# TheNeodev/RVC-MAKER

Measured on AMD Instinct MI355X. Metric: audio-seconds/sec/GPU (xRT) end-to-end VC, 48k v2; 1/2/4/8 GPU scaling, higher is better.
Workload: dtype f32-equivalent (split-fp16 3-pass MFMA for the generator's convs -- scale from the producer's published |max| -- and ResBlock pairs, split-bf16 6-pass MFMA elsewhere; f32 accumulate; RMVPE f64 with its GRU recurrence f32); 1 GPU; VC.pipeline 48k v2, ContentVec-768, rmvpe f0, one 30 s clip per GPU per step, no index, protect 0.33, clip stream (clip k+1 f0/features under clip k synthesizer); model=RVC v2 48k (NSF-HiFiGAN) + ContentVec + rmvpe, global_batch=1, seq_len=480000, parallelism=utterance-sharded x1

## Files before the change

### include/rvc_amd.h

```cpp
#ifndef RVC_AMD_H
#define RVC_AMD_H

#include <stdint.h>

#ifdef __cplusplus
extern "C" {
#endif

typedef struct ihipStream_t* rvc_stream_t;

enum { RVC_OK = 0, RVC_EINVAL = -22, RVC_EHIP = -5 };

enum {
    RVC_ACT_NONE = 0,
    RVC_ACT_LRELU = 1,
    RVC_ACT_RELU = 2,
    RVC_ACT_TANH = 3,
    RVC_ACT_GELU = 4,
    RVC_ACT_SIGMOID = 5,
    RVC_ACT_LOGCLAMP = 6,
};

const char* rvc_last_error(void);
int rvc_version(void);
// ... 3 lines not shown
#define RVC_ARITH_FP32_SA 7

typedef struct rvc_conv1d_args {
    const float* x;
    const float* w;
    const float* bias;
    const float* bias2;
    const float* res;
    float* y;
    int64_t B, Ci, Co, Lin, Lout;
    int64_t ncols;
    int64_t x_bstride, y_bstride, res_bstride, w_bstride;
    int K, stride, dil, pad, groups;
    int nphase, ostride, ooffset;
    int in_act, out_act, accumulate, _pad0;
    float in_scale, in_slope, out_slope, out_scale;
    int ntoff, wrap;
    int toff[16];
    const void* wx;
    int wx_nmf, wx_passes;
    const unsigned* amax_in;
    unsigned* amax_out;
    const float* src_x;
    const float* src_w;
    const float* src_b;
    int src_K, src_stride, src_pad, _pad1;
    int64_t src_len, src_bstride;
} rvc_conv1d_args;

int64_t rvc_conv1d_workspace_bytes(const rvc_conv1d_args* a);
int rvc_conv1d_engine(const rvc_conv1d_args* a);
int rvc_conv1d_tile(const rvc_conv1d_args* a);
int rvc_conv1d(const rvc_conv1d_args* a, void* ws, int64_t ws_bytes, rvc_stream_t stream);
void rvc_conv1d_set_probe_event(void* hip_event);
int rvc_conv1d_set_stamps(void* buf, int64_t bytes);
int rvc_resblock_set_stamps(void* buf, int64_t bytes);
int rvc_resblock_set_ylds(int on);
int rvc_resblock_set_wide64(int on);
int rvc_conv1d_set_tile_epi(int on);
int rvc_conv1d_set_swz(int on);
int rvc_conv1d_set_f16_fast(int on);
int rvc_conv1d_set_splitk_target(int target);
int rvc_stream_create_cu_mask(const uint32_t* mask, int nwords, rvc_stream_t* out);
int rvc_stream_destroy(rvc_stream_t stream);
int64_t rvc_conv1d_x6_bytes(int64_t nphase, int64_t Ci, int K, int64_t Co);
int rvc_conv1d_pack_x6(const float* w_km, int64_t nphase, int64_t Ci, int K, int64_t Co, void* out, int* nmf_out,
                       rvc_stream_t stream);
int64_t rvc_conv1d_f16_bytes(int64_t nphase, int64_t Ci, int K, int64_t Co);
int rvc_conv1d_pack_f16(const float* w_km, int64_t nphase, int64_t Ci, int K, int64_t Co, void* out, int* nmf_out,
                        rvc_stream_t stream);

typedef struct rvc_resblock_args {
    const float* x;
    float* y;
    const void* w1x;
    const float* b1;
    const void* w2x;
    const float* b2;
    int64_t C, L;
    int K, dil, nmf1, nmf2, passes, accumulate;
    float slope;
    int B;
} rvc_resblock_args;

int64_t rvc_resblock_lds_bytes(int64_t C, int K, int dil, int passes);
int rvc_resblock_pair(const rvc_resblock_args* a, rvc_stream_t stream);

typedef struct rvc_attn_args {
    const float* q;
    const float* k;
    const float* v;
    float* o;
    const float* rk;
    const float* ev;
    float* ml;
    int64_t B, H, D, T;
    int64_t ldc;
    int64_t q_hs, k_hs, v_hs, o_hs;
    int64_t q_bs, k_bs, v_bs, o_bs;
    int W, _pad0;
    float scale, _pad1;
} rvc_attn_args;

int64_t rvc_attention_workspace_bytes(const rvc_attn_args* a);
int rvc_attention(const rvc_attn_args* a, void* ws, int64_t ws_bytes, rvc_stream_t stream);
int rvc_attention_amax(const rvc_attn_args* a, unsigned* amax_out, void* ws, int64_t ws_bytes, rvc_stream_t stream);
int rvc_attention_ex(const rvc_attn_args* a, const unsigned* amax_in, unsigned* amax_out, void* ws, int64_t ws_bytes,
                     rvc_stream_t stream);
int rvc_attention_set_f16(int on);

int rvc_textenc_embed(const float* lin, const float* emb, const int64_t* pitch, float* out, int64_t B, int64_t C,
                      int64_t T, float scale, float slope, rvc_stream_t stream);
int rvc_textenc_embed_amax(const float* lin, const float* emb, const int64_t* pitch, float* out, int64_t B, int64_t C,
                           int64_t T, float scale, float slope, unsigned* amax_out, rvc_stream_t stream);
int rvc_layernorm_cf(const float* x, const float* res, const float* gamma, const float* beta, float* out, int64_t B,
                     int64_t C, int64_t T, float eps, rvc_stream_t stream);
int rvc_layernorm_cf_amax(const float* x, const float* res, const float* gamma, const float* beta, float* out,
                          int64_t B, int64_t C, int64_t T, float eps, unsigned* amax_out, rvc_stream_t stream);
int rvc_chnorm_gelu(const float* x, const float* gamma, const float* beta, float* out, int64_t B, int64_t C, int64_t L,
                    float eps, int gelu, rvc_stream_t stream);
int64_t rvc_fe0_ws_bytes(int64_t B, int64_t C, int64_t T);
int rvc_fe0_gn_gelu(const float* x, int64_t B, int64_t N, int64_t x_bstride, const float* w_km, int64_t C, int K,
                    int stride, const float* gamma, const float* beta, float* out, float eps, int gelu, void* ws,
                    int64_t ws_bytes, rvc_stream_t stream);
int rvc_fe0_gn_gelu_amax(const float* x, int64_t B, int64_t N, int64_t x_bstride, const float* w_km, int64_t C, int K,
                         int stride, const float* gamma, const float* beta, float* out, float eps, int gelu,
                         unsigned* amax_out, void* ws, int64_t ws_bytes, rvc_stream_t stream);
int rvc_prior_sample(const float* stats, const float* noise, float* zp, int64_t B, int64_t C, int64_t T, float nscale,
                     rvc_stream_t stream);
int rvc_gate(const float* a, float* out, int64_t B, int64_t H, int64_t T, rvc_stream_t stream);
int rvc_flip_channels(const float* x, float* out, int64_t B, int64_t C, int64_t T, rvc_stream_t stream);
int rvc_transpose(const float* in, float* out, int64_t B, int64_t R, int64_t C, rvc_stream_t stream);
int rvc_randn(float* out, int64_t n, uint64_t seed, uint64_t offset, rvc_stream_t stream);
int rvc_randn_ex(float* out, int64_t n, uint64_t seed, uint64_t offset, const uint64_t* seed_add,
                 rvc_stream_t stream);
int rvc_rand_triang(float* out, int64_t n, float lo, float hi, uint64_t seed, uint64_t offset,
                    const uint64_t* seed_add, rvc_stream_t stream);
int rvc_sine_source(const float* f0, const float* noise, float* har, float* work, int64_t B, int64_t T, int upp,
                    float sr, float lin_w, float lin_b, rvc_stream_t stream);

#define RVC_HARMONIC_MAX 16
#define RVC_ADAIN_BMAX 16
int rvc_rand_uniform(float* out, int64_t n, uint64_t seed, uint64_t offset, const uint64_t* seed_add,
                     rvc_stream_t stream);
int64_t rvc_harmonic_source_ws_bytes(int64_t B, int64_t T, int upp, int H);
int64_t rvc_harmonic_source_chunk(void);
int rvc_harmonic_source(const float* f0, const float* phase0, const float* noise, float* har, int64_t B, int64_t T,
                        int upp, int H, int linear, float sr, const float* lin_w, float lin_b, void* ws,
                        int64_t ws_bytes, rvc_stream_t stream);
int rvc_upsample_linear(const float* x, float* y, int64_t B, int64_t C, int64_t Lin, int r, int64_t x_bstride,
                        int64_t y_bstride, int act, float slope, rvc_stream_t stream);
int rvc_adain(const float* x, const float* noise, const float* w, float* y, int64_t B, int64_t C, int64_t L,
              float slope, float out_scale, int accumulate, const uint64_t* seeds, uint64_t offset,
              const uint64_t* seed_add, rvc_stream_t stream);

int rvc_stft_frames(const float* x, const float* win, float* framesT, int64_t N, int64_t F, int nfft, int hop,
                    rvc_stream_t stream);
int rvc_spec_mag(const float* spec, float* mag, int64_t K, int64_t F, rvc_stream_t stream);
int rvc_stft_mag(const float* x, const float* win, float* mag, int64_t B, int64_t N, int64_t F, int nfft, int hop,
                 int64_t x_bstride, int64_t mag_bstride, rvc_stream_t stream);
int rvc_mel_image(const float* mel, float* img, int64_t M, int64_t F, int64_t Tp, float scale, float shift,
                  rvc_stream_t stream);
int rvc_avgpool2(const float* in, float* out, int64_t C, int64_t H, int64_t W, rvc_stream_t stream);
// ... 301 lines not shown
```

### rvc-maker_amd/csrc/attention.hip

```cpp
#include "rvc_common.h"
#include "x6_common.h"
#include <stdlib.h>

namespace {

struct AttnParams {
    const float* q;
    const float* k;
    const float* v;
    float* o;
    const float* rk;
    float* ml;
    float* ws;
    int64_t T;
    int64_t ldc;
    int64_t q_hs, k_hs, v_hs, o_hs;
    int64_t q_bs, k_bs, v_bs, o_bs;
    int H, W, S, kps;
    float scale;
    unsigned* amax_out;
    const unsigned* amax_in;
};

template <int D>
// ... 424 lines not shown
    const float* wml = p.ws + (int64_t)gridDim.z * S * p.H * D * T;
    float m = -INFINITY;
    for (int s = 0; s < S; ++s) m = fmaxf(m, wml[(((int64_t)b * S + s) * p.H + h) * 2 * T + q]);
    float wsum = 0.f, acc[NC];
#pragma unroll
    for (int j = 0; j < NC; ++j) acc[j] = 0.f;
    for (int s = 0; s < S; ++s) {
        const int64_t bsh = ((int64_t)b * S + s) * p.H + h;
        const float w = wml[bsh * 2 * T + T + q] * expf(wml[bsh * 2 * T + q] - m);
        wsum += w;
        const float* wo = p.ws + bsh * D * T + q;
#pragma unroll
        for (int j = 0; j < NC; ++j) acc[j] += w * wo[(int64_t)(cg + 4 * j) * T];
    }
    const float inv = 1.f / wsum;
    float* O = p.o + b * p.o_bs + h * p.o_hs;
    float amx = 0.f;
    if (ok) {
#pragma unroll
        for (int j = 0; j < NC; ++j) {
            O[(int64_t)(cg + 4 * j) * p.ldc + q] = acc[j] * inv;
            amx = fmaxf(amx, fabsf(acc[j] * inv));
        }
    }
    if (p.amax_out) amax_publish(p.amax_out + (int64_t)b * RVC_AMAX_SHARDS, amx);
    if (!ok) return;
    if (p.ml && cg == 0) {
        float* ML = p.ml + ((int64_t)b * p.H + h) * 2 * T;
        ML[q] = m;
        ML[T + q] = wsum;
    }
}

constexpr int RELV_QB = 32, RELV_KW = RELV_QB + 2 * 15;
__global__ __launch_bounds__(256) void attn_relv_band_kernel(AttnParams p, const float* ev, int D) {
    constexpr int QB = RELV_QB;
    __shared__ float pb[QB][32];
    __shared__ float evs[31 * 96];
    __shared__ float qs[96][QB + 1];
    __shared__ float ks[96][RELV_KW + 1];
    const int h = blockIdx.y, b = blockIdx.z;
    const int64_t T = p.T;
    const int64_t q0 = (int64_t)blockIdx.x * QB;
    const int tid = threadIdx.x;
    const int nb = 2 * p.W + 1, kw = QB + 2 * p.W;
    const float* Q = p.q + b * p.q_bs + h * p.q_hs;
    const float* K = p.k + b * p.k_bs + h * p.k_hs;
    const float* RK = p.rk + ((int64_t)b * p.H + h) * nb * T;
    const float* ML = p.ml + ((int64_t)b * p.H + h) * 2 * T;
    float* O = p.o + b * p.o_bs + h * p.o_hs;
    for (int i = tid; i < nb * D; i += 256) evs[i] = ev[i];
    for (int i = tid; i < D * QB; i += 256) {
        const int c = i / QB, qi = i - c * QB;
        const int64_t qa = q0 + qi;
        qs[c][qi] = qa < T ? Q[(int64_t)c * p.ldc + qa] : 0.f;
    }
    for (int i = tid; i < D * kw; i += 256) {
        const int c = i / kw, ji = i - c * kw;
        const int64_t j = q0 - p.W + ji;
        ks[c][ji] = (j >= 0 && j < T) ? K[(int64_t)c * p.ldc + j] : 0.f;
    }
    __syncthreads();
    for (int i = tid; i < QB * nb; i += 256) {
        const int qi = i % QB, r = i / QB;
        const int64_t qa = q0 + qi, j = qa + r - p.W;
        float pv = 0.f;
        if (qa < T && j >= 0 && j < T) {
            float sc = 0.f;
            for (int c = 0; c < D; ++c) sc += (qs[c][qi] * p.scale) * ks[c][qi + r];
            sc += RK[(int64_t)r * T + qa];
            pv = expf(sc - ML[qa]) / ML[T + qa];
        }
        pb[qi][r] = pv;
    }
    __syncthreads();
    float amx = 0.f;
    for (int i = tid; i < QB * D; i += 256) {
        const int qi = i % QB, c = i / QB;
        const int64_t qa = q0 + qi;
        if (qa >= T) continue;
        float acc = 0.f;
        for (int r = 0; r < nb; ++r) acc += pb[qi][r] * evs[r * D + c];
        const float v = O[(int64_t)c * p.ldc + qa] + acc;
        O[(int64_t)c * p.ldc + qa] = v;
        amx = fmaxf(amx, fabsf(v));
    }
    if (p.amax_out) amax_publish_block(p.amax_out + (int64_t)b * RVC_AMAX_SHARDS, amx);
}

void attn_plan(const rvc_attn_args* a, int& S, int& kps, int qpb = 64) {
    const int64_t blocks = (int64_t)cdiv(a->T, qpb) * a->H * a->B;
    int64_t s = (512 + blocks - 1) / blocks;
    const int64_t smax = a->T / 256;
    if (s > smax) s = smax;
    if (s > 32) s = 32;
    if (s < 1) s = 1;
    kps = (int)((a->T + s - 1) / s + 63) / 64 * 64;
    S = (int)((a->T + kps - 1) / kps);
}
}

extern "C" int64_t rvc_attention_workspace_bytes(const rvc_attn_args* a) {
    if (!a || a->T <= 0 || a->H <= 0 || a->B <= 0 || (a->D != 64 && a->D != 96)) return -1;
    int S, kps, S16, kps16;
    attn_plan(a, S, kps);
    attn_plan(a, S16, kps16, af_qb(a->D));
    S = S16 > S ? S16 : S;
    if (S <= 1) return 0;
    return (int64_t)4 * a->B * S * a->H * a->T * (a->D + 2);
}

extern "C" int rvc_attention(const rvc_attn_args* a, void* ws, int64_t ws_bytes, rvc_stream_t stream) {
    return rvc_attention_amax(a, nullptr, ws, ws_bytes, stream);
}

extern "C" int rvc_attention_amax(const rvc_attn_args* a, unsigned* amax_out, void* ws, int64_t ws_bytes,
                                  rvc_stream_t stream) {
    return rvc_attention_ex(a, nullptr, amax_out, ws, ws_bytes, stream);
}

static thread_local int g_attn_f16 = -1;

extern "C" int rvc_attention_set_f16(int on) {
    g_attn_f16 = on < 0 ? -1 : (on ? 1 : 0);
    return RVC_OK;
}

extern "C" int rvc_attention_ex(const rvc_attn_args* a, const unsigned* amax_in, unsigned* amax_out, void* ws,
                                int64_t ws_bytes, rvc_stream_t stream) {
    RVC_CHECK_ARG(a && a->q && a->k && a->v && a->o && a->T > 0 && a->H > 0 && a->B > 0, "attention: bad args");
    RVC_CHECK_ARG(!amax_out || !a->rk || a->ev, "attention: amax_out with the relative band needs its value term (ev)");
    RVC_CHECK_ARG(a->D == 64 || a->D == 96, "attention: head dim %d unsupported (64, 96)", a->D);
    RVC_CHECK_ARG(!a->rk || (a->ml && a->W >= 0 && a->W <= 15), "attention: rel band needs ml and W <= 15");
    RVC_CHECK_ARG(!a->ev || (a->rk && (2 * a->W + 1) * a->D <= 31 * 96), "attention: ev band too large");
    AttnParams p;
    p.q = a->q; p.k = a->k; p.v = a->v; p.o = a->o; p.rk = a->rk; p.ml = a->ml;
    p.T = a->T; p.ldc = a->ldc ? a->ldc : a->T;
    p.q_hs = a->q_hs; p.k_hs = a->k_hs; p.v_hs = a->v_hs; p.o_hs = a->o_hs;
    p.q_bs = a->q_bs; p.k_bs = a->k_bs; p.v_bs = a->v_bs; p.o_bs = a->o_bs;
    p.H = a->H; p.W = a->W; p.scale = a->scale;
    p.amax_out = (a->rk && a->ev) ? nullptr : amax_out;
    p.amax_in = amax_in;
    static const int f16_env = getenv("RVC_ATTN_F16") ? atoi(getenv("RVC_ATTN_F16")) : 1;
    const bool f16 = amax_in && (g_attn_f16 >= 0 ? g_attn_f16 : f16_env);
    attn_plan(a, p.S, p.kps, f16 ? af_qb(a->D) : 64);
    p.ws = nullptr;
    if (p.S > 1) {
        const int64_t need = (int64_t)4 * a->B * p.S * a->H * a->T * (a->D + 2);
        RVC_CHECK_ARG(ws && ws_bytes >= need, "attention: split-KV needs %lld B of workspace (got %lld)",
                      (long long)need, (long long)ws_bytes);
        p.ws = (float*)ws;
    }
    RVC_CHECK_ARG(a->B * p.S < 65536 && a->H < 65536, "attention: grid too large");
    RVC_CHECK_ARG(!f16 || (int64_t)a->D * p.ldc < (1ll << 29), "attention: split-fp16 needs D * ldc < 2^29");
    dim3 grid(cdiv(a->T, 64), (unsigned)a->H, (unsigned)(a->B * p.S));
    hipStream_t s = (hipStream_t)stream;
    if (f16) {
        const dim3 g16(cdiv(a->T, af_qb(a->D)), (unsigned)a->H, (unsigned)(a->B * p.S));
        if (a->D == 64) hipLaunchKernelGGL(attn_f16_kernel<64>, g16, dim3(256), 0, s, p);
        else hipLaunchKernelGGL(attn_f16_kernel<96>, g16, dim3(256), 0, s, p);
    } else if (a->D == 64) hipLaunchKernelGGL(attn_fwd_kernel<64>, grid, dim3(256), 0, s, p);
    else hipLaunchKernelGGL(attn_fwd_kernel<96>, grid, dim3(256), 0, s, p);
    RVC_HIP(hipGetLastError());
    if (p.S > 1) {
        const dim3 cg(cdiv(a->T, 64), (unsigned)a->H, (unsigned)a->B);
        if (a->D == 64) hipLaunchKernelGGL(attn_combine_kernel<64>, cg, dim3(256), 0, s, p);
        else hipLaunchKernelGGL(attn_combine_kernel<96>, cg, dim3(256), 0, s, p);
        RVC_HIP(hipGetLastError());
    }
    if (a->rk && a->ev) {
        p.amax_out = amax_out;
        hipLaunchKernelGGL(attn_relv_band_kernel, dim3(cdiv(a->T, 32), (unsigned)a->H, (unsigned)a->B), dim3(256), 0,
                           s, p, a->ev, a->D);
        RVC_HIP(hipGetLastError());
    }
    return RVC_OK;
}
```

### rvc-maker_amd/csrc/conv1d.hip

```cpp
#include "rvc_common.h"
#include "x6_common.h"
#include <stdlib.h>
#include <type_traits>
#include <algorithm>

namespace {

constexpr int KCH = 32;
constexpr int NB_MAX = 16;

struct ConvParams {
    const float* x;
    const float* w;
    const float* bias;
    const float* bias2;
    const float* res;
    float* y;
    float* ws;
    int64_t B, Ci, Co, Lin, Lout, ncols;
    int64_t x_bstride, y_bstride, res_bstride, w_bstride;
    int K, stride, dil, pad, groups;
    int nphase, ostride, ooffset;
    int in_act, out_act, accumulate;
    float in_scale, in_slope, out_slope, out_scale;
    int span, span_s, rows_max;
    float inv_span;
    int mtiles_per_group, ksplit, chunks_per_split, avec;
    int ntoff, wrap;
    int toff[16];
    const uint4* wx;
    int wx_nmf, wx_nch, wx_passes;
    int rot;
    int xcd;
    int dbg;
    int tile_epi;
    const unsigned* amax_in;
    int f16_fast;
    unsigned* amax_out;
    int stagger;
    int stagger_blocks;
    int swz;
    int gx6;
#if RVC_CONV_STAMPS
    unsigned long long* stamps;
    int64_t stamp_blocks;
#endif
};

static thread_local int g_f16_fast = -1;
static thread_local int g_swz = -1;

__device__ __forceinline__ int tap_off(const ConvParams& p, int t) { return p.ntoff ? p.toff[t] : t * p.dil; }

__device__ __forceinline__ int out_pos(const ConvParams& p, int64_t n, int phase) {
    if (n >= p.ncols) return -1;
    const int t = (int)n * p.ostride + p.ooffset + phase;
    if (t < 0 || t >= (int)p.Lout) return -1;
    if (p.wrap) {
        const int row = t / p.wrap, col = t - row * p.wrap;
        if (col == 0 || col == p.wrap - 1 || row == 0 || row == (int)p.Lout / p.wrap - 1) return -(t + 2);
    }
    return t;
}

__device__ __forceinline__ float epilogue_store(const ConvParams& p, float acc, int b, int64_t m, int t) {
    const bool ok = t >= 0;
    const int64_t o = m * p.Lout + (ok ? t : 0);
    float v = acc;
    if (p.bias) v += p.bias[m];
    if (p.bias2) v += p.bias2[m];
    v = act_apply(v, p.out_act, p.out_slope) * p.out_scale;
    if (p.res) v += p.res[b * p.res_bstride + o];
    float* yb = p.y + b * p.y_bstride;
    if (p.accumulate) v += yb[o];
    if (ok) yb[o] = v;
// ... 79 lines not shown
            case RVC_ACT_LRELU: apply_act<RVC_ACT_LRELU, 1, FN>(av, p.out_slope, p.out_scale); break;
            case RVC_ACT_RELU: apply_act<RVC_ACT_RELU, 1, FN>(av, p.out_slope, p.out_scale); break;
            case RVC_ACT_TANH: apply_act<RVC_ACT_TANH, 1, FN>(av, p.out_slope, p.out_scale); break;
            case RVC_ACT_GELU: apply_act<RVC_ACT_GELU, 1, FN>(av, p.out_slope, p.out_scale); break;
            case RVC_ACT_SIGMOID: apply_act<RVC_ACT_SIGMOID, 1, FN>(av, p.out_slope, p.out_scale); break;
            case RVC_ACT_LOGCLAMP: apply_act<RVC_ACT_LOGCLAMP, 1, FN>(av, p.out_slope, p.out_scale); break;
            default: apply_act<RVC_ACT_NONE, 1, FN>(av, p.out_slope, p.out_scale); break;
        }
        if (rb2) {
#pragma unroll
            for (int r = 0; r < 4; ++r)
#pragma unroll
                for (int j = 0; j < FN; ++j) av[0][j][r] += rb2[mrow[r] * Lo + (tcol[j] >= 0 ? tcol[j] : 0)];
        }
        if (p.accumulate) {
#pragma unroll
            for (int r = 0; r < 4; ++r)
#pragma unroll
                for (int j = 0; j < FN; ++j) av[0][j][r] += yb[mrow[r] * Lo + (tcol[j] >= 0 ? tcol[j] : 0)];
        }
#pragma unroll
        for (int r = 0; r < 4; ++r)
#pragma unroll
            for (int j = 0; j < FN; ++j) {
                if (mok[r] && tcol[j] >= 0) {
                    yb[mrow[r] * Lo + tcol[j]] = av[0][j][r];
                    amx = fmaxf(amx, fabsf(av[0][j][r]));
                } else if (mok[r] && tcol[j] <= -2) {
                    yb[mrow[r] * Lo + (-tcol[j] - 2)] = 0.f;
                }
            }
    }
    if (p.amax_out) amax_publish(p.amax_out + (int64_t)b * RVC_AMAX_SHARDS, amx);
}

template <int FM, int FN, int WM, int WN>
__device__ __forceinline__ void conv_epilogue_swz(const ConvParams& p, floatx4 (&acc)[FM][FN], int lane, int wm, int wn,
                                                  int phase, int b, int g, int Cog, int m0g, int64_t n0,
                                                  const float* tb) {
    static_assert(FN % 2 == 0, "column fragments in pairs");
    constexpr int NP = FN / 2;
    const int h = lane >> 5, lc = lane & 31;
    int tcol[NP];
#pragma unroll
    for (int jp = 0; jp < NP; ++jp) tcol[jp] = out_pos(p, n0 + wn * 16 * FN + jp * 32 + lc, phase);
    float* yb = p.y + b * p.y_bstride;
    const float* rb2 = p.res ? p.res + b * p.res_bstride : nullptr;
    const int Lo = (int)p.Lout;
    float amx = 0.f;
#pragma unroll
    for (int i = 0; i < FM; ++i) {
#pragma unroll
        for (int jp = 0; jp < NP; ++jp)
#pragma unroll
            for (int r = 0; r < 4; ++r) {
                const auto sw = __builtin_amdgcn_permlane16_swap(__float_as_uint(acc[i][2 * jp][r]),
                                                                 __float_as_uint(acc[i][2 * jp + 1][r]), false, false);
                acc[i][2 * jp][r] = __uint_as_float(sw[0]);
                acc[i][2 * jp + 1][r] = __uint_as_float(sw[1]);
            }
        floatx4 (&av)[1][FN] = *reinterpret_cast<floatx4 (*)[1][FN]>(&acc[i][0]);
        int mrow[8];
        bool mok[8];
#pragma unroll
        for (int k = 0; k < 8; ++k) {
            const int mg = m0g + wm * 16 * FM + i * 16 + 8 * h + k;
// ... 172 lines not shown
                    for (int jv = 0; jv < NV; ++jv) {
                        const float v = X6_EL(kr, jv);
                        if ((okm >> jv) & 1u) {
                            *reinterpret_cast<float*>(ybase + kr * rowb + voff[jv]) = v;
                            amx = fmaxf(amx, fabsf(v));
                        }
                    }
            }
        }
    };
    if (!allok) run(std::integral_constant<int, -1>{});
    else if (rb2 && accum) run(std::integral_constant<int, 3>{});
    else if (rb2) run(std::integral_constant<int, 1>{});
    else if (accum) run(std::integral_constant<int, 2>{});
    else run(std::integral_constant<int, 0>{});
    if constexpr (PART) return;
    if (p.wrap) {
#pragma unroll 1
        for (int i = 0; i < FM; ++i) {
            const int srow = m0g + wm * 16 * FM + i * 16;
            if (srow >= Cog) continue;
#pragma unroll 1
            for (int jv = 0; jv < NV; ++jv) {
                const int t = col_pos(jv);
                if (t > -2) continue;
                for (int kr = 0; kr < NR; ++kr) yb[(int64_t)(g * Cog + srow + lrow + kr) * Lo + (-t - 2)] = 0.f;
            }
        }
    }
#undef X6_EL
    if (p.amax_out) amax_publish(p.amax_out + (int64_t)b * RVC_AMAX_SHARDS, amx);
}

template <int FM, int FN, int WM, int WN>
__global__ __launch_bounds__(256) void conv1d_mfma_kernel(ConvParams p) {
    constexpr int BM = 16 * FM * WM;
    constexpr int BN = 16 * FN * WN;
    constexpr int WS = (BM / 32) * 32 + 16 + ((BM % 32) ? 32 : 0);
    constexpr int NA = KCH * BM / 256;
    constexpr bool AVEC_OK = (NA % 4) == 0 && (BM % 4) == 0;
    extern __shared__ __attribute__((aligned(16))) float smem[];
    float* Ws = smem;
    int* koff = (int*)(smem + KCH * WS);
    float* Xs = smem + KCH * WS + KCH;

    const int tid = threadIdx.x, lane = tid & 63, wave = tid >> 6;
    const int wm = wave / WN, wn = wave % WN;
    int zb = blockIdx.z;
    const int split = zb % p.ksplit;
    zb /= p.ksplit;
    const int phase = zb % p.nphase;
    const int b = zb / p.nphase;
    const int g = blockIdx.y / p.mtiles_per_group;
    const int Cog = (int)(p.Co / p.groups);
    const int Cig = (int)(p.Ci / p.groups);
    const int m0g = (blockIdx.y % p.mtiles_per_group) * BM;
    const int64_t n0 = (int64_t)blockIdx.x * BN;

    const float* xb = p.x + b * p.x_bstride + (int64_t)g * Cig * p.Lin;
    const float* wg = p.w + b * p.w_bstride + ((int64_t)phase * p.groups + g) * (int64_t)Cig * p.K * Cog;
    const int64_t base = n0 * p.stride - p.pad;
    const int kmax = Cig * p.K;
    const int nch = (kmax + KCH - 1) / KCH;
    const int ch_beg = split * p.chunks_per_split;
    const int ch_end = min(nch, ch_beg + p.chunks_per_split);

    float ra[NA];
// ... 110 lines not shown

    const int lk = lane >> 4, ln = lane & 15;
    const float* wa = Ws + wm * (16 * FM) + ln;
    const int nb = (wn * 16 * FN + ln) * p.stride;
    const int jstep = 16 * p.stride;

    if (ch_beg < ch_end) {
        gload(ch_beg);
        sstore(ch_beg);
    }
    __syncthreads();
    for (int ch = ch_beg; ch < ch_end; ++ch) {
        const bool more = ch + 1 < ch_end;
        if (more) gload(ch + 1);
#pragma unroll
        for (int ks = 0; ks < KCH / 4; ++ks) {
            const int kk = ks * 4 + lk;
            float a[FM], bv[FN];
#pragma unroll
            for (int i = 0; i < FM; ++i) a[i] = wa[kk * WS + i * 16];
            const float* xr = Xs + koff[kk] + nb;
#pragma unroll
            for (int j = 0; j < FN; ++j) bv[j] = xr[j * jstep];
#pragma unroll
            for (int i = 0; i < FM; ++i)
#pragma unroll
                for (int j = 0; j < FN; ++j) acc[i][j] = mfma16(a[i], bv[j], acc[i][j]);
        }
        __syncthreads();
        if (more) sstore(ch + 1);
        __syncthreads();
    }

    conv_epilogue<FM, FN, WM, WN>(p, acc, lane, wm, wn, split, phase, b, g, Cog, m0g, n0);
}

constexpr int X6_NI_MAX = 6;
#ifndef RVC_CONV_ABLATIONS
#define RVC_CONV_ABLATIONS 0
#endif
constexpr bool kAblations = RVC_CONV_ABLATIONS != 0;
#ifndef X6_BPIN
#define X6_BPIN 0
#endif
#ifndef X6_NOBAR
#define X6_NOBAR 0
#endif
#if X6_NOBAR && !RVC_CONV_ABLATIONS
#error "X6_NOBAR races (wrong results): only in a -DRVC_CONV_ABLATIONS=1 profiling build"
#endif
#ifndef X6_PD8
#define X6_PD8 0
#endif
#ifndef X6_F16FAST
#define X6_F16FAST 0
#endif
#ifndef RVC_CONV_STAMPS
#define RVC_CONV_STAMPS 0
#endif
constexpr int X6_STAMP_W = 256, X6_STAMP_NC = 60;
#if RVC_CONV_STAMPS
#define X6_STAMP(slot, val)                                                                                      \
    do {                                                                                                          \
        const int64_t sb_ = (int64_t)blockIdx.x + (int64_t)gridDim.x * (blockIdx.y + (int64_t)gridDim.y * blockIdx.z); \
        if (p.stamps && lane == 0 && sb_ < p.stamp_blocks && (slot) < X6_STAMP_W)                                 \
            p.stamps[sb_ * X6_STAMP_W + (slot)] = (val);                                                         \
    } while (0)
// ... 56 lines not shown
                    v.w += rv[it].w;
                }
                if (yb_in) {
                    v.x += av[it].x;
                    v.y += av[it].y;
                    v.z += av[it].z;
                    v.w += av[it].w;
                }
                *reinterpret_cast<float4*>(dst + (int64_t)m * ld + n0 + c) = v;
                amx = fmaxf(amx, fmaxf(fmaxf(fabsf(v.x), fabsf(v.y)), fmaxf(fabsf(v.z), fabsf(v.w))));
            }
        }
        if (p.amax_out && !part) amax_publish(p.amax_out + (int64_t)b * RVC_AMAX_SHARDS, amx);
        return;
    }
    constexpr int NS = BM * BN, ITS = (NS + NT - 1) / NT;
#pragma unroll 4
    for (int it = 0; it < ITS; ++it) {
        const int idx = tid + it * NT;
        const int row = idx / BN, c = idx - row * BN;
        const int m = m0g + row;
        if (idx < NS && m < Cog && c < lim) {
            const int64_t o = (int64_t)m * ld + n0 + c;
            float v = ot[row * TS + c];
            if (rb) v += rb[o];
            if (yb_in) v += yb_in[o];
            dst[o] = v;
            amx = fmaxf(amx, fabsf(v));
        }
    }
    if (p.amax_out && !part) amax_publish(p.amax_out + (int64_t)b * RVC_AMAX_SHARDS, amx);
}

template <int FM, int FN, int WM, int WN, int X6_NI, int NP, bool F16, bool SA = false, int LF = 0>
__global__ __launch_bounds__(64 * (WM * WN + 4), (x6_min_blocks<FM, FN, WM * WN, NP>())) void conv_x6_kernel(ConvParams p) {
    static_assert(WM * WN == 4 || WM * WN == 8, "4 or 8 compute waves");
    constexpr int NCW = WM * WN;
    static_assert(NP == 6 || NP == 3 || NP == 1, "6, 3 or 1 passes");
    static_assert(!F16 || NP == 3, "split-fp16: 3 passes");
    static_assert(!SA || (NP == 6 && !F16), "split accumulators: 6-pass split-bf16");
    static_assert(LF == 0 || (F16 && WM * WN == 8), "fast-only loaders: split-fp16 on 8 compute waves");
    constexpr int NPL = NP == 6 ? 3 : (NP == 3 ? 2 : 1);
    constexpr int BM = 16 * FM * WM;
    constexpr int BN = 16 * FN * WN;
    extern __shared__ uint4 xs[];
    const int tid = threadIdx.x, lane = tid & 63;
    const int wave = __builtin_amdgcn_readfirstlane(tid >> 6);
    int bx = blockIdx.x, by = blockIdx.y, bz = blockIdx.z;
    if (p.xcd) {
        const int nx = gridDim.x, ny = gridDim.y;
        const int nwg = nx * ny * (int)gridDim.z;
        const int orig = bx + nx * (by + ny * bz);
        const int q = nwg >> 3, r = nwg & 7, xc = orig & 7;
        const int t = (xc < r ? xc * (q + 1) : r * (q + 1) + (xc - r) * q) + (orig >> 3);
        bx = t % nx;
        by = (t / nx) % ny;
        bz = t / (nx * ny);
    }
    int zb = bz;
    const int split = zb % p.ksplit;
    zb /= p.ksplit;
    const int phase = zb % p.nphase;
    const int b = zb / p.nphase;
    const int grp = p.gx6 ? phase : 0;
    const int ophase = p.gx6 ? 0 : phase;
    const int Cog = (int)p.Co;
    const int Cig = (int)p.Ci;
    const int m0g = by * BM;
// ... 365 lines not shown
            if (s0 + u < nsteps) {
                const int t = ct + rt < K ? ct + rt : ct + rt - K;
                compute(t, xs + (ci & 1) * bufsz, abuf[u]);
                if (RVC_CONV_STAMPS && wave == 0 && ct == K - 1 && ci < X6_STAMP_NC) X6_STAMP(16 + 4 * ci, X6_NOW());
                if (!X6_NOBAR && ct == K - 1) __syncthreads();
                if (RVC_CONV_STAMPS && wave == 0 && ct == K - 1 && ci < X6_STAMP_NC) X6_STAMP(16 + 4 * ci + 1, X6_NOW());
            }
            if (++ct == K) { ct = 0; ++ci; }
        }
    }
    if (wave == 0) X6_STAMP(6, X6_NOW());
    if constexpr (SA) {
#pragma unroll
        for (int i = 0; i < FM; ++i)
#pragma unroll
            for (int j = 0; j < FN; ++j)
#pragma unroll
                for (int r = 0; r < 4; ++r) acc[i][j][r] += acc_lo[i][j][r];
    }
    if (kAblations && (p.dbg & 1)) {
        if (acc[0][0][0] == 1234.5f) p.y[lane] = acc[FM - 1][FN - 1][3];
        return;
    }
    if constexpr (F16) {
#pragma unroll
        for (int i = 0; i < FM; ++i)
#pragma unroll
            for (int r = 0; r < 4; ++r) {
                const float f = etab[wm * 16 * FM + i * 16 + lg * 4 + r] * tile_rs;
#pragma unroll
                for (int j = 0; j < FN; ++j) acc[i][j][r] *= f;
            }
    }
    if (BN <= 128 && p.tile_epi) {
        float* ot = reinterpret_cast<float*>(xs);
        constexpr int TS = BN + 4;
#pragma unroll
        for (int i = 0; i < FM; ++i) {
            floatx4 (&av)[1][FN] = *reinterpret_cast<floatx4 (*)[1][FN]>(&acc[i][0]);
            if (p.ksplit == 1) {
#pragma unroll
                for (int r = 0; r < 4; ++r) {
                    const int mg = m0g + wm * 16 * FM + i * 16 + lg * 4 + r;
                    const float bs = epi_bias<true, BM>(p, etab, wm * 16 * FM + i * 16 + lg * 4 + r, 0);
#pragma unroll
                    for (int j = 0; j < FN; ++j) av[0][j][r] += bs;
                }
                switch (p.out_act) {
                    case RVC_ACT_LRELU: apply_act<RVC_ACT_LRELU, 1, FN>(av, p.out_slope, p.out_scale); break;
                    case RVC_ACT_RELU: apply_act<RVC_ACT_RELU, 1, FN>(av, p.out_slope, p.out_scale); break;
                    case RVC_ACT_TANH: apply_act<RVC_ACT_TANH, 1, FN>(av, p.out_slope, p.out_scale); break;
                    case RVC_ACT_GELU: apply_act<RVC_ACT_GELU, 1, FN>(av, p.out_slope, p.out_scale); break;
                    case RVC_ACT_SIGMOID: apply_act<RVC_ACT_SIGMOID, 1, FN>(av, p.out_slope, p.out_scale); break;
                    case RVC_ACT_LOGCLAMP: apply_act<RVC_ACT_LOGCLAMP, 1, FN>(av, p.out_slope, p.out_scale); break;
                    default: apply_act<RVC_ACT_NONE, 1, FN>(av, p.out_slope, p.out_scale); break;
                }
            }
        }
        auto put = [&](int row0) __attribute__((always_inline)) {
#pragma unroll
            for (int i = 0; i < FM; ++i)
#pragma unroll
                for (int r = 0; r < 4; ++r)
#pragma unroll
                    for (int j = 0; j < FN; ++j)
                        ot[(wm * 16 * FM - row0 + i * 16 + lg * 4 + r) * TS + wn * 16 * FN + j * 16 + ln] = acc[i][j][r];
        };
// ... 65 lines not shown
        float x = s[r];
        if (p.bias) x += p.bias[m];
        if (p.bias2) x += p.bias2[m];
        v[r] = act_apply(x, p.out_act, p.out_slope) * p.out_scale;
    }
    if (p.res) {
        float rr[RED_ROWS];
#pragma unroll
        for (int r = 0; r < RED_ROWS; ++r) rr[r] = p.res[b * p.res_bstride + o[r]];
#pragma unroll
        for (int r = 0; r < RED_ROWS; ++r) v[r] += rr[r];
    }
    float* yb = p.y + b * p.y_bstride;
    if (p.accumulate) {
        float aa[RED_ROWS];
#pragma unroll
        for (int r = 0; r < RED_ROWS; ++r) aa[r] = yb[o[r]];
#pragma unroll
        for (int r = 0; r < RED_ROWS; ++r) v[r] += aa[r];
    }
    float amx = 0.f;
#pragma unroll
    for (int r = 0; r < RED_ROWS; ++r) {
        if (r < nr) {
            if (ok) {
                yb[o[r]] = v[r];
                amx = fmaxf(amx, fabsf(v[r]));
            } else if (t <= -2) {
                yb[(m0 + r) * Lo + (-t - 2)] = 0.f;
            }
        }
    }
    if (p.amax_out) amax_publish_block(p.amax_out + (int64_t)b * RVC_AMAX_SHARDS, amx);
}

struct SrcParams {
    float* y;
    const float* x;
    const float* w;
    const float* b;
    unsigned* amax_out;
    int64_t Co, Lout, len, xbs, ybs;
    int K, stride, pad, span;
};
constexpr int SRC_T = 256, SRC_M = 16;

__global__ __launch_bounds__(SRC_T) void src_add_kernel(SrcParams p) {
    extern __shared__ __attribute__((aligned(16))) float smem_src[];
    float* sw = smem_src;
    float* sx = smem_src + p.K * SRC_M;
    const int b = blockIdx.z;
    const int64_t t0 = (int64_t)blockIdx.x * SRC_T;
    const int64_t q0 = t0 * p.stride - p.pad;
    const float* xb = p.x + b * p.xbs;
    const int m0 = blockIdx.y * SRC_M;
    const int nm = p.Co - m0 < SRC_M ? (int)(p.Co - m0) : SRC_M;
    for (int i = threadIdx.x; i < p.K * SRC_M; i += SRC_T) {
        const int k = i / SRC_M, mi = i - k * SRC_M;
        sw[i] = mi < nm ? p.w[(int64_t)k * p.Co + m0 + mi] : 0.f;
    }
    for (int i = threadIdx.x; i < p.span; i += SRC_T) {
        const int64_t q = q0 + i;
        sx[i] = (q >= 0 && q < p.len) ? xb[q] : 0.f;
    }
    __syncthreads();
    const int64_t t = t0 + threadIdx.x;
// ... 84 lines not shown
unsigned long long* g_stamps = nullptr;
int64_t g_stamp_blocks = 0;
#endif

void fill_common(const rvc_conv1d_args* a, ConvParams& p) {
    p.x = a->x; p.w = a->w; p.bias = a->bias; p.bias2 = a->bias2; p.res = a->res; p.y = a->y; p.ws = nullptr;
    p.B = a->B; p.Ci = a->Ci; p.Co = a->Co; p.Lin = a->Lin; p.Lout = a->Lout;
    p.ncols = a->ncols > 0 ? a->ncols : a->Lout;
    p.x_bstride = a->x_bstride ? a->x_bstride : a->Ci * a->Lin;
    p.y_bstride = a->y_bstride ? a->y_bstride : a->Co * a->Lout;
    p.res_bstride = a->res_bstride ? a->res_bstride : a->Co * a->Lout;
    p.w_bstride = a->w_bstride;
    p.K = a->K; p.stride = a->stride; p.dil = a->dil; p.pad = a->pad; p.groups = a->groups;
    p.nphase = a->nphase; p.ostride = a->ostride; p.ooffset = a->ooffset;
    p.in_act = a->in_act; p.out_act = a->out_act; p.accumulate = a->accumulate;
    p.in_scale = a->in_scale; p.in_slope = a->in_slope; p.out_slope = a->out_slope; p.out_scale = a->out_scale;
    p.ntoff = a->ntoff; p.wrap = a->wrap;
    for (int i = 0; i < 16; ++i) p.toff[i] = a->ntoff ? a->toff[i] : 0;
    p.wx = nullptr;
    p.wx_nmf = p.wx_nch = 0;
    p.wx_passes = a->wx_passes == 0 ? 6 : a->wx_passes;
    static const int dbg = getenv("RVC_CONV_DEBUG") ? atoi(getenv("RVC_CONV_DEBUG")) : 0;
    p.dbg = dbg;
    p.tile_epi = 0;
    p.amax_in = a->amax_in;
    p.amax_out = a->amax_out;
    static const int f16fast = getenv("RVC_X6_F16FAST") ? atoi(getenv("RVC_X6_F16FAST")) : 1;
    p.f16_fast = g_f16_fast >= 0 ? g_f16_fast : f16fast;
    p.stagger = 0;
    p.stagger_blocks = 0;
    static const int swz_env = getenv("RVC_X6_SWZ") ? atoi(getenv("RVC_X6_SWZ")) : 1;
    p.swz = g_swz >= 0 ? g_swz : swz_env;
    p.gx6 = 0;
#if RVC_CONV_STAMPS
    p.stamps = g_stamps;
    p.stamp_blocks = g_stamp_blocks;
#endif
    static const int rot = getenv("RVC_X6_ROT") ? atoi(getenv("RVC_X6_ROT")) : 0;
    p.rot = rot;
    static const int xcd = getenv("RVC_X6_XCD") ? atoi(getenv("RVC_X6_XCD")) : 1;
    p.xcd = xcd;
}

int num_cus() {
    static const int n = [] {
        int dev = 0, cus = 0;
        if (hipGetDevice(&dev) != hipSuccess ||
            hipDeviceGetAttribute(&cus, hipDeviceAttributeMultiprocessorCount, dev) != hipSuccess || cus <= 0)
            cus = 256;
        return cus;
    }();
    return n;
}

static thread_local int g_splitk_target = -1;
static thread_local int g_tile_epi = -1;

void split_k(ConvParams& p, int64_t tiles, int nch, int per_cu = 2) {
    static const int env_target = getenv("RVC_SPLITK_TILES") ? atoi(getenv("RVC_SPLITK_TILES")) : 256;
    static const int occ_aware = getenv("RVC_X6_SPLIT_OCC") ? atoi(getenv("RVC_X6_SPLIT_OCC")) : 1;
    int target = g_splitk_target >= 0 ? g_splitk_target : env_target;
    if (occ_aware && per_cu == 1 && g_splitk_target < 0) target /= 2;
    int ks = 1;
    if (tiles < target && nch >= 4) {
        ks = (int)((target + tiles - 1) / tiles);
        if (ks > 16) ks = 16;
// ... 4 lines not shown
    p.ksplit = (nch + p.chunks_per_split - 1) / p.chunks_per_split;
}

constexpr int X6_BN = 128;

int max_tap_off(const rvc_conv1d_args* a) {
    if (!a->ntoff) return (a->K - 1) * a->dil;
    int m = 0;
    for (int i = 0; i < a->ntoff && i < 16; ++i) m = a->toff[i] > m ? a->toff[i] : m;
    return m;
}

constexpr int X6_K_MAX = 64;
constexpr int X6_K_MAX_GROUPED = 128;

bool x6_eligible(const rvc_conv1d_args* a) {
    static const int s2 = getenv("RVC_X6_STRIDE2") ? atoi(getenv("RVC_X6_STRIDE2")) : 1;
    static const int k1 = getenv("RVC_X6_K1") ? atoi(getenv("RVC_X6_K1")) : 1;
    if (a->K == 1 && !k1) return false;
    static const int grouped = getenv("RVC_X6_GROUPED") ? atoi(getenv("RVC_X6_GROUPED")) : 1;
    const bool grp_ok = a->groups == 1 ||
                        (grouped && a->stride == 1 && a->nphase == 1 && a->ostride == 1 && a->ooffset == 0 &&
                         !a->ntoff && !a->wrap && !a->src_x && a->Ci % a->groups == 0 && a->Co % a->groups == 0);
    return a->wx && a->Lin < (1 << 24) &&
           (a->stride == 1 || (s2 && a->stride == 2 && a->Ci >= 32 && !a->ntoff)) && grp_ok &&
           a->w_bstride == 0 && (!a->ntoff || a->ntoff == a->K) &&
           a->K <= (a->groups == 1 ? X6_K_MAX : X6_K_MAX_GROUPED) &&
           (X6_BN - 1) * a->stride + max_tap_off(a) + 1 <= 64 * X6_NI_MAX - 2 && a->wx_nmf % 8 == 0 &&
           (int64_t)a->wx_nmf * 16 >= a->Co / a->groups && (a->wx_passes == 0 || a->wx_passes == 6 ||
                                                a->wx_passes == RVC_ARITH_FP32_SA || a->wx_passes == 3 ||
                                                a->wx_passes == 1 || a->wx_passes == RVC_ARITH_F16X3);
}

int plan(const rvc_conv1d_args* a, ConvParams& p, Cfg& cfg, dim3& grid, size_t& lds) {
    RVC_CHECK_ARG(a && a->x && a->w && a->y, "conv1d: null pointer");
    RVC_CHECK_ARG(a->B > 0 && a->Ci > 0 && a->Co > 0 && a->K > 0 && a->Lin > 0 && a->Lout > 0,
                  "conv1d: bad sizes B=%lld Ci=%lld Co=%lld K=%d Lin=%lld Lout=%lld", (long long)a->B,
                  (long long)a->Ci, (long long)a->Co, a->K, (long long)a->Lin, (long long)a->Lout);
    RVC_CHECK_ARG(a->groups >= 1 && a->Ci % a->groups == 0 && a->Co % a->groups == 0, "conv1d: bad groups");
    RVC_CHECK_ARG(a->stride >= 1 && a->dil >= 1 && a->nphase >= 1 && a->ostride >= 1, "conv1d: bad stride/dil");
    RVC_CHECK_ARG(a->Co * a->Lout < (1ll << 31) && a->Ci * a->Lin < (1ll << 31) && a->Lin + a->pad < (1ll << 30),
                  "conv1d: per-batch tensor exceeds 2^31 elements (use the batch dimension)");
    const int64_t Cog = a->Co / a->groups;
    const int64_t Cig = a->Ci / a->groups;
    const int64_t ncols = a->ncols > 0 ? a->ncols : a->Lout;
    fill_common(a, p);
    RVC_CHECK_ARG(!a->src_x || (a->src_w && a->src_K > 0 && a->src_K <= 4096 && a->src_stride > 0 && a->src_pad >= 0 &&
                                a->src_len > 0 && a->src_bstride >= 0 && !a->wrap),
                  "conv1d: bad fused source conv (src_K=%d src_stride=%d src_pad=%d src_len=%lld)", a->src_K,
                  a->src_stride, a->src_pad, (long long)a->src_len);
    RVC_CHECK_ARG(!a->src_x || ((int64_t)255 * a->src_stride + 17 * a->src_K) * 4 <= 64 * 1024,
                  "conv1d: source conv span too large (stride %d, K %d)", a->src_stride, a->src_K);
    if (a->ntoff) {
        RVC_CHECK_ARG(a->ntoff == a->K && a->K <= 16, "conv1d: toff needs ntoff == K <= 16");
        for (int i = 0; i < a->K; ++i) RVC_CHECK_ARG(a->toff[i] >= 0, "conv1d: negative tap offset");
    }

    if (x6_eligible(a)) {
        cfg.x6 = true;
        static const int w8 = getenv("RVC_X6_W8") ? atoi(getenv("RVC_X6_W8")) : 1;
        const int np = a->wx_passes == 0 || a->wx_passes == RVC_ARITH_FP32_SA ? 6 : a->wx_passes;
        static const int bn256 = getenv("RVC_X6_BN256") ? atoi(getenv("RVC_X6_BN256")) : 1;
        auto round_eff = [](int64_t t) {
            const int64_t n = num_cus();
            return (double)t / (double)(((t + n - 1) / n) * n);
        };
        const int64_t rows128 = (Cog + 127) / 128, nb = a->B * a->nphase;
        const bool fills256 = round_eff(rows128 * ((ncols + 255) / 256) * nb) >=
                              round_eff(rows128 * ((ncols + 127) / 128) * nb) - 0.05;
        if (Cog > 64 && w8 && bn256 && a->stride == 1 && 255 + max_tap_off(a) + 1 <= 64 * X6_NI_MAX - 2 &&
            Cog % 16 == 0 && a->Lout < (1ll << 26) && ncols < (1ll << 26) &&
            (bn256 == 2 || np == RVC_ARITH_F16X3) && (fills256 || bn256 == 3))
            cfg = {2, 8, 4, 2, true};
        else if (Cog > 64 && w8) cfg = {2, 4, 4, 2, true};
        else if (Cog > 64) cfg = {4, 4, 2, 2, true};
        else if (Cog > 32 && w8 && np >= 3) cfg = {2, 2, 2, 4, true};
        else if (Cog > 32) cfg = {2, 4, 2, 2, true};
        else if (Cog > 16) cfg = {2, 2, 1, 4, true};
        else cfg = {1, 2, 1, 4, true};
        RVC_CHECK_ARG(a->wx_passes != RVC_ARITH_FP32_SA || x6_sa_tile(cfg.FM, cfg.FN, cfg.WM, cfg.WN),
                      "conv1d: RVC_ARITH_FP32_SA has no split-accumulator kernel for the %dx%d tile on %d waves "
                      "(engine switches changed?)", 16 * cfg.FM * cfg.WM, 16 * cfg.FN * cfg.WN, cfg.WM * cfg.WN);
        const int BM = 16 * cfg.FM * cfg.WM, BN = 16 * cfg.FN * cfg.WN;
        p.span = (BN - 1) * a->stride + max_tap_off(a) + 1;
        p.span_s = p.span;
        p.rows_max = 0;
        p.inv_span = 1.0f / (float)p.span;
        p.avec = 0;
        p.wx = (const uint4*)a->wx;
        p.wx_nmf = a->wx_nmf;
        p.wx_nch = (int)((Cig + 31) / 32);
        p.mtiles_per_group = (int)((Cog + BM - 1) / BM);
        const int64_t tiles = (int64_t)p.mtiles_per_group * ((ncols + BN - 1) / BN) * a->B * a->nphase * a->groups;
        split_k(p, tiles, p.wx_nch, cfg.WM * cfg.WN == 8 ? 1 : 2);
        if (a->groups > 1) {
            p.gx6 = 1;
            p.nphase = a->groups;
            p.Ci = Cig;
            p.Co = Cog;
            p.chunks_per_split = p.wx_nch;
            p.ksplit = 1;
        }
        lds = (size_t)2 * (p.wx_passes == 6 || p.wx_passes == RVC_ARITH_FP32_SA ? 3 : (p.wx_passes == 1 ? 1 : 2)) *
              p.span * 64 + 16;
        static const int tepi_env = getenv("RVC_X6_TILE_EPI") ? atoi(getenv("RVC_X6_TILE_EPI")) : 0;
        const int tepi = g_tile_epi >= 0 ? g_tile_epi : tepi_env;
        const size_t tile_bytes = (size_t)BM * (BN + 4) * 4;
        const bool plain = a->nphase == 1 && a->ostride == 1 && a->ooffset == 0 && !a->wrap && !(p.dbg & 1) &&
                           BN <= 128;
        p.tile_epi = !(tepi && plain && a->groups == 1) ? 0
                     : tile_bytes <= lds ? 1 : (cfg.WM % 2 == 0 && tile_bytes / 2 <= lds) ? 2 : 0;
        lds += (size_t)3 * BM * 4;
        grid = dim3(cdiv(ncols, BN), (unsigned)p.mtiles_per_group, (unsigned)(a->B * p.nphase * p.ksplit));
        RVC_CHECK_ARG(grid.y < 65536 && grid.z < 65536, "conv1d: grid too large");
        static const int stagger = getenv("RVC_X6_STAGGER") ? atoi(getenv("RVC_X6_STAGGER")) : 0;
        static const int stagger_rounds = getenv("RVC_X6_STAGGER_ROUNDS") ? atoi(getenv("RVC_X6_STAGGER_ROUNDS")) : 2;
        const int64_t nblk = (int64_t)grid.x * grid.y * grid.z;
        if (stagger > 0 && nblk >= stagger_rounds * (int64_t)num_cus()) {
            p.stagger = stagger;
            p.stagger_blocks = num_cus();
        }
        return RVC_OK;
    }

    if (Cog % 48 == 0 && Cog % 64 != 0) cfg = {3, 1, 1, 4, false};
    else if (Cog <= 16) cfg = {1, 4, 1, 4, false};
    else if (Cog <= 32) cfg = {2, 4, 1, 4, false};
    else if (Cog <= 64 || Cog % 128 != 0) cfg = {2, 4, 2, 2, false};
    else cfg = {4, 4, 2, 2, false};
    int BM = 16 * cfg.FM * cfg.WM, BN = 16 * cfg.FN * cfg.WN;

    const int maxoff = max_tap_off(a);
    int rows_max = (KCH % a->K == 0) ? KCH / a->K : (KCH - 1) / a->K + 2;
    if (rows_max > Cig) rows_max = (int)Cig;
    int span = (BN - 1) * a->stride + maxoff + 1;
    while ((int64_t)rows_max * span > 256 * NB_MAX && cfg.FN > 2) {
        cfg.FN /= 2;
        BN = 16 * cfg.FN * cfg.WN;
        span = (BN - 1) * a->stride + maxoff + 1;
    }
    RVC_CHECK_ARG((int64_t)rows_max * span <= 256 * NB_MAX, "conv1d: staged tile too large (rows %d x span %d)",
                  rows_max, span);
    p.span = span;
// ... 170 lines not shown
}

static thread_local hipEvent_t g_probe_event = nullptr;

extern "C" void rvc_conv1d_set_probe_event(void* hip_event) { g_probe_event = (hipEvent_t)hip_event; }

extern "C" int rvc_conv1d_set_f16_fast(int on) {
    g_f16_fast = on < 0 ? -1 : (on ? 1 : 0);
    return RVC_OK;
}

extern "C" int rvc_conv1d_set_swz(int on) {
    g_swz = on < 0 ? -1 : (on ? 1 : 0);
    return RVC_OK;
}

extern "C" int rvc_conv1d_set_tile_epi(int on) {
    g_tile_epi = on < 0 ? -1 : (on ? 1 : 0);
    return RVC_OK;
}

extern "C" int rvc_conv1d_set_stamps(void* buf, int64_t bytes) {
#if RVC_CONV_STAMPS
    g_stamps = (unsigned long long*)buf;
    g_stamp_blocks = buf ? bytes / (8 * X6_STAMP_W) : 0;
    return 0;
#else
    (void)buf;
    (void)bytes;
    return -1;
#endif
}

extern "C" int rvc_conv1d(const rvc_conv1d_args* a, void* ws, int64_t ws_bytes, rvc_stream_t stream) {
    ConvParams p;
    Cfg cfg;
    dim3 grid;
    size_t lds;
    int rc = plan(a, p, cfg, grid, lds);
    if (rc != RVC_OK) return rc;
    if (p.ksplit > 1) {
        const int64_t need = (int64_t)p.ksplit * p.B * p.nphase * p.Co * p.ncols * 4;
        RVC_CHECK_ARG(ws && ws_bytes >= need, "conv1d: split-K needs %lld B of workspace (got %lld)",
                      (long long)need, (long long)ws_bytes);
        p.ws = (float*)ws;
    }
    hipStream_t s = (hipStream_t)stream;
    if (a->src_x) p.amax_out = nullptr;
    hipError_t e;
    if (cfg.x6) {
        if (cfg.WM == 4 && cfg.FN == 8) e = launch_x6<2, 8, 4, 2>(p, grid, lds, s);
        else if (cfg.WM == 4) e = launch_x6<2, 4, 4, 2>(p, grid, lds, s);
        else if (cfg.WM == 2 && cfg.WN == 4) e = launch_x6<2, 2, 2, 4>(p, grid, lds, s);
        else if (cfg.FM == 4) e = launch_x6<4, 4, 2, 2>(p, grid, lds, s);
        else if (cfg.WM == 2) e = launch_x6<2, 4, 2, 2>(p, grid, lds, s);
        else if (cfg.FM == 2) e = launch_x6<2, 2, 1, 4>(p, grid, lds, s);
        else e = launch_x6<1, 2, 1, 4>(p, grid, lds, s);
    } else if (cfg.FM == 3) e = launch<3, 1, 1, 4>(p, grid, lds, s);
    else if (cfg.FM == 1 && cfg.FN == 4) e = launch<1, 4, 1, 4>(p, grid, lds, s);
    else if (cfg.FM == 1) e = launch<1, 2, 1, 4>(p, grid, lds, s);
    else if (cfg.WM == 1 && cfg.FN == 4) e = launch<2, 4, 1, 4>(p, grid, lds, s);
    else if (cfg.WM == 1) e = launch<2, 2, 1, 4>(p, grid, lds, s);
    else if (cfg.FM == 4 && cfg.FN == 4) e = launch<4, 4, 2, 2>(p, grid, lds, s);
    else if (cfg.FM == 4) e = launch<4, 2, 2, 2>(p, grid, lds, s);
    else if (cfg.FN == 4) e = launch<2, 4, 2, 2>(p, grid, lds, s);
    else e = launch<2, 2, 2, 2>(p, grid, lds, s);
    RVC_HIP(e);
    if (g_probe_event) RVC_HIP(hipEventRecord(g_probe_event, s));
    if (p.ksplit > 1) {
        hipLaunchKernelGGL(conv_splitk_reduce,
                           dim3(cdiv(p.ncols, 256), (unsigned)cdiv(p.Co, RED_ROWS), (unsigned)(p.B * p.nphase)),
                           dim3(256), 0, s, p);
        RVC_HIP(hipGetLastError());
    }
    if (a->src_x) {
        SrcParams q;
        q.y = a->y;
        q.x = a->src_x;
        q.w = a->src_w;
        q.b = a->src_b;
// ... 17 lines not shown
```

### rvc-maker_amd/csrc/elementwise.hip

```cpp
#include "rvc_common.h"

RVC_DEV void philox(uint32_t c[4], uint32_t k0, uint32_t k1) {
#pragma unroll
    for (int i = 0; i < 10; ++i) {
        uint64_t p0 = (uint64_t)0xD2511F53u * c[0];
        uint64_t p1 = (uint64_t)0xCD9E8D57u * c[2];
        uint32_t n0 = (uint32_t)(p1 >> 32) ^ c[1] ^ k0;
        uint32_t n2 = (uint32_t)(p0 >> 32) ^ c[3] ^ k1;
        c[0] = n0; c[1] = (uint32_t)p1; c[2] = n2; c[3] = (uint32_t)p0;
        k0 += 0x9E3779B9u; k1 += 0xBB67AE85u;
    }
}

__global__ void rand_kernel(float* out, int64_t n, uint64_t seed, uint64_t offset, const uint64_t* seed_add, int kind,
                            float lo, float hi) {
    int64_t i = (int64_t)blockIdx.x * blockDim.x + threadIdx.x;
    int64_t base = i * 4;
    if (base >= n) return;
    if (seed_add) seed += *seed_add;
    uint64_t ctr = (uint64_t)i + offset;
    uint32_t c[4] = {(uint32_t)ctr, (uint32_t)(ctr >> 32), 0x7A3Bu, 0x52u};
    philox(c, (uint32_t)seed, (uint32_t)(seed >> 32));
    float r[4];
    if (kind == 0) {
// ... 86 lines not shown
    const float* sb = stats + (int64_t)b * 2 * C * T;
    float m = sb[(int64_t)c * T + t];
    float lg = sb[(int64_t)(c + C) * T + t];
    int64_t o = ((int64_t)b * C + c) * T + t;
    zp[o] = (m + expf(lg) * noise[o] * nscale);
}

extern "C" int rvc_prior_sample(const float* stats, const float* noise, float* zp, int64_t B, int64_t C, int64_t T,
                                float nscale, rvc_stream_t stream) {
    RVC_CHECK_ARG(stats && noise && zp && B > 0 && C > 0 && T > 0, "prior_sample: bad args");
    hipLaunchKernelGGL(prior_kernel, dim3(cdiv(T, 256), (unsigned)C, (unsigned)B), dim3(256), 0, (hipStream_t)stream,
                       stats, noise, zp, (int)C, T, nscale);
    RVC_HIP(hipGetLastError());
    return RVC_OK;
}

__global__ void gate_kernel(const float* a, float* out, int H, int64_t T) {
    int64_t t = (int64_t)blockIdx.x * blockDim.x + threadIdx.x;
    int c = blockIdx.y, b = blockIdx.z;
    if (t >= T) return;
    const float* ab = a + (int64_t)b * 2 * H * T;
    float x0 = ab[(int64_t)c * T + t], x1 = ab[(int64_t)(c + H) * T + t];
    out[((int64_t)b * H + c) * T + t] = tanhf(x0) * (1.f / (1.f + expf(-x1)));
}

extern "C" int rvc_gate(const float* a, float* out, int64_t B, int64_t H, int64_t T, rvc_stream_t stream) {
    RVC_CHECK_ARG(a && out && B > 0 && H > 0 && T > 0, "gate: bad args");
    hipLaunchKernelGGL(gate_kernel, dim3(cdiv(T, 256), (unsigned)H, (unsigned)B), dim3(256), 0, (hipStream_t)stream,
                       a, out, (int)H, T);
    RVC_HIP(hipGetLastError());
    return RVC_OK;
}

__global__ void flip_kernel(const float* x, float* out, int C, int64_t T) {
    int64_t t = (int64_t)blockIdx.x * blockDim.x + threadIdx.x;
    int c = blockIdx.y, b = blockIdx.z;
    if (t >= T) return;
    out[((int64_t)b * C + c) * T + t] = x[((int64_t)b * C + (C - 1 - c)) * T + t];
}

extern "C" int rvc_flip_channels(const float* x, float* out, int64_t B, int64_t C, int64_t T, rvc_stream_t stream) {
    RVC_CHECK_ARG(x && out && x != out && B > 0 && C > 0 && T > 0, "flip: bad args");
    hipLaunchKernelGGL(flip_kernel, dim3(cdiv(T, 256), (unsigned)C, (unsigned)B), dim3(256), 0, (hipStream_t)stream,
                       x, out, (int)C, T);
    RVC_HIP(hipGetLastError());
    return RVC_OK;
}

__global__ void transpose_kernel(const float* in, float* out, int64_t R, int64_t C) {
    __shared__ float tile[32][33];
    int b = blockIdx.z;
    const float* ib = in + (int64_t)b * R * C;
    float* ob = out + (int64_t)b * R * C;
    int64_t c0 = (int64_t)blockIdx.x * 32, r0 = (int64_t)blockIdx.y * 32;
    int tx = threadIdx.x & 31, ty = threadIdx.x >> 5;
    for (int k = ty; k < 32; k += 8) {
        int64_t r = r0 + k, c = c0 + tx;
        tile[k][tx] = (r < R && c < C) ? ib[r * C + c] : 0.f;
    }
    __syncthreads();
    for (int k = ty; k < 32; k += 8) {
        int64_t c = c0 + k, r = r0 + tx;
        if (c < C && r < R) ob[c * R + r] = tile[tx][k];
    }
}

// ... 135 lines not shown
```

### rvc-maker_amd/csrc/model_common.h

```cpp
#pragma once
#include <hip/hip_runtime_api.h>
#include <math.h>
#include <stdint.h>
#include <stdlib.h>
#include <string.h>

#include <map>
#include <string>
#include <vector>

#include "../../include/rvc_amd.h"

void rvc_set_error(const char* fmt, ...);

#define MCHECK(cond, ...)               \
    do {                                \
        if (!(cond)) {                  \
            rvc_set_error(__VA_ARGS__); \
            return RVC_EINVAL;          \
        }                               \
    } while (0)
#define MHIP(call)                                                  \
    do {                                                            \
        hipError_t e_ = (call);                                     \
        if (e_ != hipSuccess) {                                     \
            rvc_set_error("%s: %s", #call, hipGetErrorString(e_)); \
            return RVC_EHIP;                                        \
        }                                                           \
    } while (0)
#define MTRY(call)                     \
    do {                               \
        int rc_ = (call);              \
        if (rc_ != RVC_OK) return rc_; \
    } while (0)

struct Synth;
struct ContentVec;
struct Rmvpe;
struct Crepe;
struct VcState;

struct rvc_ctx {
    int device = 0;
    int prec = RVC_PREC_FP32;
    int rm_prec = RVC_PREC_FP64;
    bool x6 = true, f16mix = true, fused_rb = true;
    bool amax = true;
    bool amax_f16all = true;
    bool cv_amax = true;
    bool amax_ups = true;
    bool amax_s2 = true;
    bool fe_amax = true;
    bool fused_noise = false;
    bool attn_f16 = true;
    bool te_amax = false;
    bool flow_amax = false;
    Synth* syn = nullptr;
    ContentVec* cv = nullptr;
    Rmvpe* rm = nullptr;
    Crepe* cr = nullptr;
    VcState* vc = nullptr;
};

void synth_delete(Synth* s);
void contentvec_delete(ContentVec* m);
void rmvpe_delete(Rmvpe* m);
void crepe_delete(Crepe* m);
void vc_delete(VcState* v);

int synth_run_cf(rvc_ctx* c, const float* phone_cf, const int64_t* pitch, const float* pitchf, int64_t T, int64_t sid,
                 uint64_t seed, float* wav, hipStream_t s);
bool synth_info(const rvc_ctx* c, int* emb_dim, int* upp);
int contentvec_cf(rvc_ctx* c, const float* wav, int64_t N, int out_layer, int final_proj, float* feats_cf,
                  hipStream_t s);

namespace rvcm {

struct HostT {
    std::vector<float> v;
    std::vector<int64_t> shape;
    int64_t dim(int i) const { return i < (int)shape.size() ? shape[i] : 1; }
};

inline float half_to_float(uint16_t h) {
    const uint32_t s = (uint32_t)(h >> 15) << 31, e = (h >> 10) & 31, m = h & 1023;
    uint32_t bits;
    if (e == 0) {
        if (m == 0) {
            bits = s;
// ... 216 lines not shown
    m.ws_bytes = bytes;
    return RVC_OK;
}

inline int ensure_arena(ModelBase& m, int64_t floats, hipStream_t s) {
    if (floats <= m.arena_floats) return RVC_OK;
    if (m.arena) {
        MHIP(hipStreamSynchronize(s));
        MHIP(hipFree(m.arena));
        m.arena = nullptr;
        m.arena_floats = 0;
    }
    MHIP(hipMalloc((void**)&m.arena, floats * 4));
    m.arena_floats = floats;
    return RVC_OK;
}

struct CallOpts {
    const float* bias2 = nullptr;
    const float* res = nullptr;
    int stride = 1, pad = 0, dil = 1;
    int64_t Lout = -1;
    int in_act = RVC_ACT_NONE, out_act = RVC_ACT_NONE, accumulate = 0;
    float in_slope = 0.f, in_scale = 1.f, out_slope = 0.f, out_scale = 1.f;
    int64_t B = 1, x_bstride = 0, y_bstride = 0, res_bstride = 0;
    int ntoff = 0, wrap = 0;
    int toff[16] = {0};
    const unsigned* amax_in = nullptr;
    unsigned* amax_out = nullptr;
    const ConvW* src = nullptr;
    const float* src_x = nullptr;
    int src_stride = 1, src_pad = 0;
    int64_t src_len = 0;
};

inline int conv(rvc_ctx* c, ModelBase& m, const ConvW& cw, const float* x, int64_t Lin, float* y, const CallOpts& o,
                hipStream_t s) {
    rvc_conv1d_args a;
    memset(&a, 0, sizeof(a));
    a.x = x;
    a.w = cw.w;
    a.bias = cw.b;
    a.bias2 = o.bias2;
    a.res = o.res;
    a.y = y;
    a.B = o.B;
    a.Ci = cw.Ci;
    a.Co = cw.Co;
    a.Lin = Lin;
    a.x_bstride = o.x_bstride;
    a.y_bstride = o.y_bstride;
    a.res_bstride = o.res_bstride;
    a.groups = cw.groups;
    a.in_act = o.in_act;
    a.in_slope = o.in_slope;
    a.in_scale = o.in_scale;
    a.out_act = o.out_act;
    a.out_slope = o.out_slope;
    a.out_scale = o.out_scale;
    a.accumulate = o.accumulate;
    a.K = cw.K;
    a.ntoff = o.ntoff;
    a.wrap = o.wrap;
    for (int i = 0; i < o.ntoff; ++i) a.toff[i] = o.toff[i];
    a.amax_in = o.amax_in;
    a.amax_out = o.amax_out;
    if (o.src) {
        a.src_x = o.src_x;
        a.src_w = o.src->w;
        a.src_b = o.src->b;
        a.src_K = o.src->K;
        a.src_stride = o.src_stride;
        a.src_pad = o.src_pad;
        a.src_len = o.src_len;
        a.src_bstride = o.src_len;
    }
    int stride = o.stride;
    if (cw.nphase > 1) {
        const int64_t Lout = (Lin - 1) * cw.u - 2 * cw.tpad + cw.Kfull;
        a.Lout = Lout;
        a.ncols = (Lout - 1 + cw.tpad) / cw.u + 1;
        a.stride = 1;
        a.pad = cw.K - 1;
        a.dil = 1;
        a.nphase = cw.u;
        a.ostride = cw.u;
        a.ooffset = -cw.tpad;
        stride = 1;
    } else {
        a.Lout = o.Lout >= 0 ? o.Lout : (Lin + 2 * o.pad - o.dil * (cw.K - 1) - 1) / o.stride + 1;
        a.stride = o.stride;
        a.pad = o.pad;
        a.dil = o.dil;
        a.nphase = 1;
        a.ostride = 1;
    }
    if (cw.wx_bf) {
        const int passes = conv_passes(c, cw.K, cw.Ci / cw.groups, stride, o.ntoff > 0, o.amax_in != nullptr);
        a.wx = passes == RVC_ARITH_F16X3 ? cw.wx_hf : cw.wx_bf;
        a.wx_nmf = cw.nmf;
        a.wx_passes = passes;
    }
    const int64_t need = rvc_conv1d_workspace_bytes(&a);
    if (need < 0) return RVC_EINVAL;
    MTRY(ensure_ws(m, need, s));
    return rvc_conv1d(&a, need ? m.ws : nullptr, need, s);
}

struct Scratch {
    float* base = nullptr;
    int64_t off = 0;
    bool dry = true;
    float* take(int64_t n) {
        float* p = dry ? (float*)(uintptr_t)(256 + off * 4) : base + off;
        off += (n + 63) & ~int64_t(63);
        return p;
    }
};
#define RUN(call)              \
    do {                       \
        if (!sc.dry) MTRY(call); \
    } while (0)

struct Plan {
    int64_t off = 0;
    int64_t take(int64_t n) {
        const int64_t o = off;
        off += (n + 63) & ~int64_t(63);
        return o;
    }
};

inline bool env_on(const char* name) {
    const char* v = getenv(name);
    return !(v && strcmp(v, "0") == 0);
}

inline bool env_set(const char* name) {
// ... 6 lines not shown
```

### rvc-maker_amd/csrc/rvc_common.h

```cpp
#pragma once
#include <hip/hip_runtime.h>
#include <stdint.h>
#include <math.h>

#include "../../include/rvc_amd.h"

typedef float floatx4 __attribute__((ext_vector_type(4)));

#define RVC_DEV __device__ __forceinline__

RVC_DEV floatx4 mfma16(float a, float b, floatx4 c) {
    return __builtin_amdgcn_mfma_f32_16x16x4f32(a, b, c, 0, 0, 0);
}

RVC_DEV float act_apply(float v, int act, float slope) {
    switch (act) {
        case RVC_ACT_LRELU: return v >= 0.f ? v : v * slope;
        case RVC_ACT_RELU: return v > 0.f ? v : 0.f;
        case RVC_ACT_TANH: return tanhf(v);
        case RVC_ACT_GELU: return 0.5f * v * (1.f + erff(v * 0.70710678118654752440f));
        case RVC_ACT_SIGMOID: return 1.f / (1.f + expf(-v));
        case RVC_ACT_LOGCLAMP: return logf(fmaxf(v, slope));
        default: return v;
    }
}

RVC_DEV float wave_sum(float v) {
#pragma unroll
    for (int o = 32; o > 0; o >>= 1) v += __shfl_xor(v, o, 64);
    return v;
}

RVC_DEV float wave_max(float v) {
#pragma unroll
    for (int o = 32; o > 0; o >>= 1) v = fmaxf(v, __shfl_xor(v, o, 64));
    return v;
}

RVC_DEV void amax_publish(unsigned* amax_out, float m) {
    m = wave_max(m);
    const unsigned shard = (blockIdx.x + 7u * blockIdx.y + 13u * blockIdx.z + (threadIdx.x >> 6)) % RVC_AMAX_SHARDS;
    if ((threadIdx.x & 63) == 0) atomicMax(amax_out + shard, __float_as_uint(m));
}

RVC_DEV void amax_publish_block(unsigned* amax_out, float m) {
    __shared__ float wmax_[16];
    m = wave_max(m);
    if ((threadIdx.x & 63) == 0) wmax_[threadIdx.x >> 6] = m;
    __syncthreads();
    if (threadIdx.x == 0) {
        float bm = 0.f;
        for (int w = 0; w < (int)((blockDim.x + 63) >> 6); ++w) bm = fmaxf(bm, wmax_[w]);
        const unsigned shard = (blockIdx.x + 7u * blockIdx.y + 13u * blockIdx.z) % RVC_AMAX_SHARDS;
        atomicMax(amax_out + shard, __float_as_uint(bm));
    }
}

typedef const __attribute__((address_space(4))) unsigned* amax_const_ptr;
// ... 64 lines not shown
```

### rvc-maker_amd/csrc/rvc_model.cpp

```cpp
#include "model_common.h"

using namespace rvcm;

namespace synthm {

constexpr float kLreluSlope = 0.1f;

struct Pair {
    int d;
    ConvW c1, c2;
};

struct Layer {
    ConvW qkv, relk, o, ffn1, ffn2;
    float *ev = nullptr, *ln1g = nullptr, *ln1b = nullptr, *ln2g = nullptr, *ln2b = nullptr;
};

struct Flow {
    ConvW pre, post;
    ConvW ins[3], rs_a[2], rs_b[3];
};

}

struct Synth : ModelBase {
    rvc_synth_cfg cfg{};
    int emb_dim = 0, upp = 1, kc = 0;
    ConvW emb_phone, proj, cond, conv_pre, conv_post;
    float *emb_pitch = nullptr, *emb_g = nullptr;
    int64_t n_spk = 0;
    std::vector<synthm::Layer> layers;
    synthm::Flow flows[4];
    float lin_w = 0, lin_b = 0;
    std::vector<ConvW> ups;
    std::vector<ConvW> noise;
    std::vector<int> noise_stride, noise_pad, chans;
    std::vector<std::vector<std::vector<synthm::Pair>>> res;
};


void synth_delete(Synth* s) {
    if (!s) return;
    s->release();
    delete s;
}

namespace synthm {

int64_t convT_out_len(const ConvW& cw, int64_t Lin) { return (Lin - 1) * cw.u - 2 * cw.tpad + cw.Kfull; }

int rb_passes(const rvc_ctx* c, int K) {
    static const int kmin = getenv("RVC_AMD_RB_F16_KMIN") ? atoi(getenv("RVC_AMD_RB_F16_KMIN")) : 3;
    if (c->prec == RVC_PREC_FP32 && c->f16mix && K >= kmin) return RVC_ARITH_F16X3;
    return base_passes(c);
}

bool rb_pass_ok(int passes) { return passes == 6 || passes == 3 || passes == 1 || passes == RVC_ARITH_F16X3; }

bool resblock_fusable(const rvc_ctx* c, const ConvW& c1, const ConvW& c2, int d) {
    static const bool rb128 = getenv("RVC_AMD_FUSED_RB128") && atoi(getenv("RVC_AMD_FUSED_RB128")) != 0;
    const int passes = rb_passes(c, c1.K);
    const bool chans = c1.Co == 32 || c1.Co == 64 || (c1.Co == 128 && rb128 && passes != 6);
    return c->fused_rb && rb_pass_ok(passes) && c1.wx_bf && c2.wx_bf && c1.Ci == c1.Co && c2.Ci == c2.Co &&
           c1.Co == c2.Co && chans && c1.K == c2.K && c1.K % 2 == 1 && c1.K <= 15 && (c1.K - 1) * d <= 64;
}
// ... 150 lines not shown
        o.amax_in = te_cell;
        MTRY(conv(c, S, S.proj, x, T, stats, o, s));
    }
    float* zp = A + bf.zp;
    if (!z_noise) {
        float* zn = A + bf.znoise;
        MTRY(rvc_randn_ex(zn, I * T, seed, 0, nullptr, s));
        z_noise = zn;
    }
    MTRY(rvc_prior_sample(stats, z_noise, zp, 1, I, T, 0.66666f, s));
    float *h = A + bf.h, *acts = A + bf.acts, *outacc = A + bf.outacc, *xin = A + bf.xin;
    float* bufs[2] = {A + bf.fb0, A + bf.fb1};
    float* xf_cur = zp;
    const unsigned* unit = fcell(1 + 5 * nl);
    const unsigned* post_cell = nullptr;
    for (int f = 3, n = 0; f >= 0; --f, ++n) {
        const Flow& F = S.flows[f];
        unsigned* c_h[3] = {fcell(2 + 5 * nl + 5 * n), fcell(3 + 5 * nl + 5 * n), fcell(4 + 5 * nl + 5 * n)};
        unsigned *c_acc = fcell(5 + 5 * nl + 5 * n), *c_post = fcell(6 + 5 * nl + 5 * n);
        float* xf = (xf_cur != bufs[0]) ? bufs[0] : bufs[1];
        MTRY(rvc_flip_channels(xf_cur, xf, 1, I, T, s));
        float *x0 = xf, *x1 = xf + half * T;
        {
            CallOpts o;
            o.amax_in = post_cell;
            o.amax_out = c_h[0];
            MTRY(conv(c, S, F.pre, x0, T, h, o, s));
        }
        for (int l = 0; l < 3; ++l) {
            CallOpts oi;
            oi.pad = (F.ins[l].K - 1) / 2;
            oi.bias2 = gc + (int64_t)f * 6 * H + (int64_t)l * 2 * H;
            oi.amax_in = c_h[l];
            MTRY(conv(c, S, F.ins[l], h, T, xin, oi, s));
            MTRY(rvc_gate(xin, acts, 1, H, T, s));
            if (l < 2) {
                CallOpts ra;
                ra.res = h;
                ra.amax_in = unit;
                ra.amax_out = c_h[l + 1];
                MTRY(conv(c, S, F.rs_a[l], acts, T, h, ra, s));
                CallOpts rb;
                rb.accumulate = l > 0;
                rb.amax_in = unit;
                MTRY(conv(c, S, F.rs_b[l], acts, T, outacc, rb, s));
            } else {
                CallOpts rb;
                rb.accumulate = 1;
                rb.amax_in = unit;
                rb.amax_out = c_acc;
                MTRY(conv(c, S, F.rs_b[l], acts, T, outacc, rb, s));
            }
        }
        CallOpts po;
        po.res = x1;
        po.out_scale = -1.f;
        po.amax_in = c_acc;
        po.amax_out = c_post;
        MTRY(conv(c, S, F.post, outacc, T, x1, po, s));
        post_cell = c_post;
        xf_cur = xf;
    }
    const float* z = xf_cur;
    float *har = A + bf.har, *work = A + bf.work;
    if (!sine_noise) {
        float* sn = A + bf.snoise;
        MTRY(rvc_randn_ex(sn, L, seed, (uint64_t)1 << 40, nullptr, s));
        sine_noise = sn;
    }
// ... 121 lines not shown
    CallOpts op;
    op.pad = 3;
    op.in_act = RVC_ACT_LRELU;
    op.in_slope = 0.01f;
    op.in_scale = scale_in;
    op.out_act = RVC_ACT_TANH;
    return conv(c, S, S.conv_post, xcur, Lcur, wav, op, s);
}

}

using namespace synthm;


extern "C" int rvc_ctx_create(int hip_device, rvc_ctx** out) {
    MCHECK(out, "rvc_ctx_create: null out");
    *out = nullptr;
    MHIP(hipSetDevice(hip_device));
    rvc_ctx* c = new rvc_ctx();
    c->device = hip_device;
    c->x6 = env_on("RVC_AMD_X6");
    c->f16mix = env_on("RVC_AMD_F16MIX");
    c->fused_rb = env_on("RVC_AMD_FUSED_RB");
    c->amax = env_on("RVC_AMD_AMAX");
    c->amax_f16all = env_on("RVC_AMD_AMAX_F16ALL");
    c->cv_amax = env_on("RVC_AMD_CV_AMAX");
    c->amax_ups = env_on("RVC_AMD_AMAX_UPS");
    c->amax_s2 = env_on("RVC_AMD_AMAX_S2");
    c->fe_amax = env_on("RVC_AMD_FE_AMAX");
    c->fused_noise = env_set("RVC_AMD_FUSED_NOISE");
    c->attn_f16 = env_on("RVC_AMD_ATTN_F16");
    c->te_amax = env_set("RVC_AMD_TE_AMAX");
    c->flow_amax = env_set("RVC_AMD_FLOW_AMAX");
    *out = c;
    return RVC_OK;
}

extern "C" void rvc_ctx_destroy(rvc_ctx* c) {
    if (!c) return;
    if (hipSetDevice(c->device) == hipSuccess) {
        (void)hipDeviceSynchronize();
        synth_delete(c->syn);
        vc_delete(c->vc);
        contentvec_delete(c->cv);
        rmvpe_delete(c->rm);
        crepe_delete(c->cr);
    }
    delete c;
}

extern "C" int rvc_ctx_set_precision(rvc_ctx* c, int prec) {
    MCHECK(c, "rvc_ctx_set_precision: null ctx");
    MCHECK(prec == RVC_PREC_FP32 || prec == RVC_PREC_BF16 || prec == RVC_PREC_BF16X3 || prec == RVC_PREC_FP32X6 ||
               prec == RVC_PREC_FP32SA || prec == RVC_PREC_F16X3,
           "rvc_ctx_set_precision: unknown precision %d", prec);
    c->prec = prec;
    return RVC_OK;
}

extern "C" int64_t rvc_synth_out_len(const rvc_ctx* c, int64_t T) {
    if (!c || !c->syn || !c->syn->loaded || T <= 0) return -1;
    return T * c->syn->upp;
}

namespace {
int expect(const HostT& t, const std::string& name, int64_t d0, int64_t d1 = -1, int64_t d2 = -1, int ndim = -1) {
// ... 76 lines not shown
        MTRY(expect(w, p + "emb_rel_v", 1, 21, S.kc));
        MTRY(upload(S, w.v, &Ly.ev));
        GET(p + "conv_o.weight", w);
        GET(p + "conv_o.bias", b);
        MTRY(expect(w, p + "conv_o.weight", H, H, 1));
        MTRY(make_conv(c, S, w, &b, Ly.o));
        const std::string si = std::to_string(i);
        GET("enc_p.encoder.norm_layers_1." + si + ".gamma", w);
        MTRY(expect(w, "norm_layers_1." + si + ".gamma", H, -1, -1, 1));
        MTRY(upload(S, w.v, &Ly.ln1g));
        GET("enc_p.encoder.norm_layers_1." + si + ".beta", w);
        MTRY(expect(w, "norm_layers_1." + si + ".beta", H, -1, -1, 1));
        MTRY(upload(S, w.v, &Ly.ln1b));
        GET("enc_p.encoder.ffn_layers." + si + ".conv_1.weight", w);
        GET("enc_p.encoder.ffn_layers." + si + ".conv_1.bias", b);
        MTRY(expect(w, "ffn_layers." + si + ".conv_1.weight", g.filter_channels, H, g.kernel_size));
        MTRY(make_conv(c, S, w, &b, Ly.ffn1));
        GET("enc_p.encoder.ffn_layers." + si + ".conv_2.weight", w);
        GET("enc_p.encoder.ffn_layers." + si + ".conv_2.bias", b);
        MTRY(expect(w, "ffn_layers." + si + ".conv_2.weight", H, g.filter_channels, g.kernel_size));
        MTRY(make_conv(c, S, w, &b, Ly.ffn2));
        GET("enc_p.encoder.norm_layers_2." + si + ".gamma", w);
        MTRY(expect(w, "norm_layers_2." + si + ".gamma", H, -1, -1, 1));
        MTRY(upload(S, w.v, &Ly.ln2g));
        GET("enc_p.encoder.norm_layers_2." + si + ".beta", w);
        MTRY(expect(w, "norm_layers_2." + si + ".beta", H, -1, -1, 1));
        MTRY(upload(S, w.v, &Ly.ln2b));
        S.layers.push_back(Ly);
    }
    GET("enc_p.proj.weight", w);
    GET("enc_p.proj.bias", b);
    MTRY(expect(w, "enc_p.proj.weight", 2 * g.inter_channels, H, 1));
    MTRY(make_conv(c, S, w, &b, S.proj));
    {
        HostT cw, cb;
        for (int f = 0; f <= 4; ++f) {
            const std::string p = f < 4 ? "flow.flows." + std::to_string(2 * f) + ".enc.cond_layer." : "dec.cond.";
            GET(p + "weight", w);
            GET(p + "bias", b);
            MTRY(expect(w, p + "weight", f < 4 ? 2 * H * 3 : g.upsample_initial_channel, g.gin_channels, 1));
            if (f == 0) {
                cw = w;
                cb = b;
            } else {
                cw.v.insert(cw.v.end(), w.v.begin(), w.v.end());
                cw.shape[0] += w.dim(0);
                cb.v.insert(cb.v.end(), b.v.begin(), b.v.end());
            }
        }
        MTRY(make_conv(c, S, cw, &cb, S.cond));
    }
    GET("emb_g.weight", w);
    MCHECK(w.dim(1) == g.gin_channels, "rvc_load_synth: emb_g width %lld != gin_channels %d", (long long)w.dim(1),
           g.gin_channels);
    S.n_spk = w.dim(0);
    MTRY(upload(S, w.v, &S.emb_g));
    for (int f = 0; f < 4; ++f) {
        Flow& F = S.flows[f];
        const std::string p = "flow.flows." + std::to_string(2 * f) + ".";
        GET(p + "pre.weight", w);
        GET(p + "pre.bias", b);
        MTRY(expect(w, p + "pre.weight", H, g.inter_channels / 2, 1));
        MTRY(make_conv(c, S, w, &b, F.pre));
        GET(p + "post.weight", w);
        GET(p + "post.bias", b);
        MTRY(expect(w, p + "post.weight", g.inter_channels / 2, H, 1));
        MTRY(make_conv(c, S, w, &b, F.post));
        for (int l = 0; l < 3; ++l) {
            const std::string sl = std::to_string(l);
            GET(p + "enc.in_layers." + sl + ".weight", w);
            GET(p + "enc.in_layers." + sl + ".bias", b);
            MTRY(expect(w, p + "enc.in_layers." + sl + ".weight", 2 * H, H, 5));
            MTRY(make_conv(c, S, w, &b, F.ins[l]));
            GET(p + "enc.res_skip_layers." + sl + ".weight", w);
            GET(p + "enc.res_skip_layers." + sl + ".bias", b);
            MTRY(expect(w, p + "enc.res_skip_layers." + sl + ".weight", l < 2 ? 2 * H : H, H, 1));
            if (l < 2) {
                const int64_t inner = (int64_t)w.v.size() / w.dim(0);
                HostT wa = w, wb = w, ba = b, bb = b;
                wa.v.assign(w.v.begin(), w.v.begin() + H * inner);
                wa.shape[0] = H;
                wb.v.assign(w.v.begin() + H * inner, w.v.end());
                wb.shape[0] = w.dim(0) - H;
                ba.v.assign(b.v.begin(), b.v.begin() + H);
                bb.v.assign(b.v.begin() + H, b.v.end());
                MTRY(make_conv(c, S, wa, &ba, F.rs_a[l]));
                MTRY(make_conv(c, S, wb, &bb, F.rs_b[l]));
            } else {
                MTRY(make_conv(c, S, w, &b, F.rs_b[l]));
            }
        }
    }
    GET("dec.m_source.l_linear.weight", w);
    GET("dec.m_source.l_linear.bias", b);
    MTRY(expect(w, "dec.m_source.l_linear.weight", 1, 1, -1, 2));
    MTRY(expect(b, "dec.m_source.l_linear.bias", 1, -1, -1, 1));
    S.lin_w = w.v[0];
    S.lin_b = b.v[0];
    GET("dec.conv_pre.weight", w);
    GET("dec.conv_pre.bias", b);
    MTRY(expect(w, "dec.conv_pre.weight", g.upsample_initial_channel, g.inter_channels, 7));
    MTRY(make_conv(c, S, w, &b, S.conv_pre));
    const int nup = g.n_upsamples;
    S.ups.resize(nup);
    S.noise.resize(nup);
    S.res.resize(nup);
    for (int i = 0; i < nup; ++i) {
        const int u = g.upsample_rates[i], k = g.upsample_kernel_sizes[i];
        S.chans.push_back(g.upsample_initial_channel >> (i + 1));
        const std::string si = std::to_string(i);
        GET("dec.ups." + si + ".weight", w);
        GET("dec.ups." + si + ".bias", b);
        const int ch = g.upsample_initial_channel >> (i + 1);
        MTRY(expect(w, "dec.ups." + si + ".weight", 2 * ch, ch, k));
        MTRY(expect(b, "dec.ups." + si + ".bias", ch, -1, -1, 1));
        MTRY(make_convT(c, S, w, b, u, (k - u) / 2, S.ups[i]));
        int st = 1;
        for (int j = i + 1; j < nup; ++j) st *= g.upsample_rates[j];
        const int kn = st == 1 ? 1 : st * 2 - st % 2;
        S.noise_stride.push_back(st);
// ... 65 lines not shown
```

### rvc-maker_amd/rvc_amd/_lib.py

```python
from __future__ import annotations

import ctypes
import os
from ctypes import POINTER, c_double, c_float, c_int, c_int64, c_uint64, c_void_p

LIB_PATH = os.environ.get("RVC_AMD_LIB") or os.path.join(
    os.path.dirname(os.path.dirname(os.path.abspath(__file__))), "lib", "librvc_amd.so")

ACT_NONE, ACT_LRELU, ACT_RELU, ACT_TANH, ACT_GELU, ACT_SIGMOID, ACT_LOGCLAMP = 0, 1, 2, 3, 4, 5, 6


class Conv1dArgs(ctypes.Structure):
    _fields_ = [("x", c_void_p), ("w", c_void_p), ("bias", c_void_p), ("bias2", c_void_p), ("res", c_void_p),
                ("y", c_void_p),
                ("B", c_int64), ("Ci", c_int64), ("Co", c_int64), ("Lin", c_int64), ("Lout", c_int64),
                ("ncols", c_int64), ("x_bstride", c_int64), ("y_bstride", c_int64), ("res_bstride", c_int64),
                ("w_bstride", c_int64),
                ("K", c_int), ("stride", c_int), ("dil", c_int), ("pad", c_int), ("groups", c_int),
                ("nphase", c_int), ("ostride", c_int), ("ooffset", c_int),
                ("in_act", c_int), ("out_act", c_int), ("accumulate", c_int), ("_pad0", c_int),
                ("in_scale", c_float), ("in_slope", c_float), ("out_slope", c_float), ("out_scale", c_float),
                ("ntoff", c_int), ("wrap", c_int), ("toff", c_int * 16),
                ("wx", c_void_p), ("wx_nmf", c_int), ("wx_passes", c_int),
                ("amax_in", c_void_p), ("amax_out", c_void_p),
                ("src_x", c_void_p), ("src_w", c_void_p), ("src_b", c_void_p),
                ("src_K", c_int), ("src_stride", c_int), ("src_pad", c_int), ("_pad1", c_int),
                ("src_len", c_int64), ("src_bstride", c_int64)]


class Conv64Args(ctypes.Structure):
    _fields_ = [("x", c_void_p), ("w", c_void_p), ("bias", c_void_p), ("res", c_void_p), ("y", c_void_p),
                ("B", c_int64), ("Ci", c_int64), ("Co", c_int64), ("Lin", c_int64), ("Lout", c_int64),
                ("x_bstride", c_int64), ("y_bstride", c_int64), ("res_bstride", c_int64),
                ("K", c_int), ("pad", c_int), ("out_act", c_int), ("y_f32", c_int), ("out_slope", c_double),
                ("ntoff", c_int), ("wrap", c_int), ("toff", c_int * 16),
                ("w_bstride", c_int64), ("w_bmod", c_int), ("_pad0", c_int)]


class Wino64Args(ctypes.Structure):
    _fields_ = [("x", c_void_p), ("v", c_void_p), ("bias", c_void_p), ("res", c_void_p), ("y", c_void_p),
                ("B", c_int64), ("Ci", c_int64), ("Co", c_int64), ("H", c_int64), ("W", c_int64),
                ("x_bstride", c_int64), ("y_bstride", c_int64), ("res_bstride", c_int64),
                ("out_act", c_int), ("y_f32", c_int)]


class AttnArgs(ctypes.Structure):
    _fields_ = [("q", c_void_p), ("k", c_void_p), ("v", c_void_p), ("o", c_void_p), ("rk", c_void_p),
                ("ev", c_void_p), ("ml", c_void_p),
                ("B", c_int64), ("H", c_int64), ("D", c_int64), ("T", c_int64), ("ldc", c_int64),
                ("q_hs", c_int64), ("k_hs", c_int64), ("v_hs", c_int64), ("o_hs", c_int64),
                ("q_bs", c_int64), ("k_bs", c_int64), ("v_bs", c_int64), ("o_bs", c_int64),
                ("W", c_int), ("_pad0", c_int), ("scale", c_float), ("_pad1", c_float)]


class F0Post(ctypes.Structure):
    _fields_ = [("autotune", c_int), ("_pad0", c_int), ("strength", c_double), ("rep", c_void_p),
                ("rep_off", c_int64), ("rep_len", c_int64)]


class F0Track(ctypes.Structure):
    _fields_ = [("f0", c_void_p), ("n", c_int64), ("is_f64", c_int), ("_pad0", c_int)]

# ... 25 lines not shown
    _fields_ = [("inter_channels", c_int), ("hidden_channels", c_int), ("filter_channels", c_int), ("n_heads", c_int),
                ("n_layers", c_int), ("kernel_size", c_int), ("n_resblocks", c_int), ("n_dilations", c_int),
                ("resblock_kernel_sizes", c_int * 4), ("resblock_dilation_sizes", (c_int * 4) * 4),
                ("n_upsamples", c_int), ("upsample_rates", c_int * 8), ("upsample_kernel_sizes", c_int * 8),
                ("upsample_initial_channel", c_int), ("spk_embed_dim", c_int), ("gin_channels", c_int), ("sr", c_int)]


class ContentVecCfg(ctypes.Structure):
    _fields_ = [("encoder_embed_dim", c_int), ("encoder_attention_heads", c_int), ("conv_pos_groups", c_int),
                ("_pad0", c_int)]


class VcArgs(ctypes.Structure):
    _fields_ = [("sid", c_int64), ("pitch_shift", c_double), ("protect", c_float), ("version", c_int),
                ("x_pad", c_int), ("x_max", c_int), ("tgt_sr", c_int), ("_pad0", c_int), ("index_rate", c_double), ("seed", c_uint64)]


class VcOpts(ctypes.Structure):
    _fields_ = [("f0_method", c_int), ("f0_autotune", c_int), ("f0_autotune_strength", c_double),
                ("f0_file", c_void_p), ("f0_file_rows", c_int64), ("volume_envelope", c_double),
                ("crepe_dither", c_void_p)]


class IvfIndex(ctypes.Structure):
    _fields_ = [("d", c_int64), ("nlist", c_int64), ("ntotal", c_int64), ("nprobe", c_int), ("_pad0", c_int),
                ("centroids", c_void_p), ("list_off", c_void_p), ("codes", c_void_p), ("ids", c_void_p),
                ("big", c_void_p)]


SIGNATURES = {
    "rvc_last_error": [],
    "rvc_version": [],
    "rvc_conv1d": [POINTER(Conv1dArgs), c_void_p, c_int64, c_void_p],
    "rvc_conv1d_workspace_bytes": [POINTER(Conv1dArgs)],
    "rvc_conv1d_set_probe_event": [c_void_p],
    "rvc_conv1d_set_stamps": [c_void_p, c_int64],
    "rvc_resblock_set_stamps": [c_void_p, c_int64],
    "rvc_resblock_set_ylds": [c_int],
    "rvc_resblock_set_wide64": [c_int],
    "rvc_conv1d_set_tile_epi": [c_int],
    "rvc_conv1d_set_swz": [c_int],
    "rvc_conv1d_set_f16_fast": [c_int],
    "rvc_bigru64_set_f32": [c_int],
    "rvc_conv1d_set_splitk_target": [c_int],
    "rvc_stream_create_cu_mask": [c_void_p, c_int, POINTER(c_void_p)],
    "rvc_stream_destroy": [c_void_p],
    "rvc_conv1d_engine": [POINTER(Conv1dArgs)],
    "rvc_conv1d_tile": [POINTER(Conv1dArgs)],
    "rvc_conv1d_x6_bytes": [c_int64, c_int64, c_int, c_int64],
    "rvc_conv1d_pack_x6": [c_void_p, c_int64, c_int64, c_int, c_int64, c_void_p, POINTER(c_int), c_void_p],
    "rvc_conv1d_f16_bytes": [c_int64, c_int64, c_int, c_int64],
    "rvc_pm_frames": [c_int64],
    "rvc_pm_work_bytes": [c_int64],
    "rvc_pm_f0": [c_void_p, c_int64, c_void_p, c_void_p, c_void_p, c_int64, c_void_p, c_void_p],
    "rvc_pm_post": [c_void_p, c_int64, c_int64, ctypes.c_double, c_void_p, c_void_p, c_void_p, c_void_p],
    "rvc_swipe_frames": [c_int64],
    "rvc_swipe_work_bytes": [c_int64],
    "rvc_swipe_tables_bytes": [],
    "rvc_swipe_table_dims": [c_int, c_int, POINTER(c_int64)],
    "rvc_swipe_tables": [c_void_p, c_int64],
    "rvc_swipe_strength": [c_void_p, c_int64, c_void_p, c_void_p, c_int64, c_void_p, c_void_p],
    "rvc_swipe_pick": [c_void_p, c_int64, c_void_p, c_void_p, c_void_p],
    "rvc_swipe_post": [c_void_p, c_int64, c_float, POINTER(F0Post), c_void_p, c_void_p, c_void_p],
    "rvc_abs_quantile_work_bytes": [],
    "rvc_abs_quantile": [c_void_p, c_int64, c_void_p, c_int64, c_void_p, c_void_p],
    "rvc_div_scalar": [c_void_p, c_int64, c_void_p, c_void_p, c_void_p],
    "rvc_f0_mix": [POINTER(F0Track), c_int, c_int64, c_void_p, c_void_p],
    "rvc_fcpe_mel": [c_void_p, c_void_p, c_void_p, c_int64, c_int64, c_void_p],
    "rvc_groupnorm_work_bytes": [c_int64, c_int],
    "rvc_groupnorm_act": [c_void_p, c_void_p, c_void_p, c_void_p, c_int64, c_int64, c_int64, c_int, c_float, c_float,
                          c_void_p, c_int64, c_void_p],
    "rvc_glu_dwconv_silu": [c_void_p, c_void_p, c_void_p, c_void_p, c_int64, c_int64, c_int64, c_int, c_void_p],
    "rvc_fcpe_decode": [c_void_p, c_void_p, c_void_p, c_int64, c_int64, c_int64, c_float, c_float, c_float, c_void_p],
    "rvc_fcpe_post_work_bytes": [c_int64],
    "rvc_fcpe_post": [c_void_p, c_int64, c_int64, c_int, c_int, c_void_p, c_int64, c_void_p, c_void_p],
    "rvc_conv1d_pack_f16": [c_void_p, c_int64, c_int64, c_int, c_int64, c_void_p, POINTER(c_int), c_void_p],
    "rvc_attention_workspace_bytes": [POINTER(AttnArgs)],
    "rvc_attention": [POINTER(AttnArgs), c_void_p, c_int64, c_void_p],
    "rvc_attention_amax": [POINTER(AttnArgs), c_void_p, c_void_p, c_int64, c_void_p],
    "rvc_attention_ex": [POINTER(AttnArgs), c_void_p, c_void_p, c_void_p, c_int64, c_void_p],
    "rvc_attention_set_f16": [c_int],
    "rvc_layernorm_cf_amax": [c_void_p, c_void_p, c_void_p, c_void_p, c_void_p, c_int64, c_int64, c_int64, c_float,
                              c_void_p, c_void_p],
    "rvc_textenc_embed": [c_void_p, c_void_p, c_void_p, c_void_p, c_int64, c_int64, c_int64, c_float, c_float,
                          c_void_p],
    "rvc_textenc_embed_amax": [c_void_p, c_void_p, c_void_p, c_void_p, c_int64, c_int64, c_int64, c_float, c_float,
                               c_void_p, c_void_p],
    "rvc_layernorm_cf": [c_void_p, c_void_p, c_void_p, c_void_p, c_void_p, c_int64, c_int64, c_int64, c_float,
                         c_void_p],
    "rvc_chnorm_gelu": [c_void_p, c_void_p, c_void_p, c_void_p, c_int64, c_int64, c_int64, c_float, c_int, c_void_p],
    "rvc_fe0_ws_bytes": [c_int64, c_int64, c_int64],
    "rvc_fe0_gn_gelu": [c_void_p, c_int64, c_int64, c_int64, c_void_p, c_int64, c_int, c_int, c_void_p, c_void_p, c_void_p,
                        c_float, c_int, c_void_p, c_int64, c_void_p],
    "rvc_fe0_gn_gelu_amax": [c_void_p, c_int64, c_int64, c_int64, c_void_p, c_int64, c_int, c_int, c_void_p, c_void_p,
                             c_void_p, c_float, c_int, c_void_p, c_void_p, c_int64, c_void_p],
    "rvc_prior_sample": [c_void_p, c_void_p, c_void_p, c_int64, c_int64, c_int64, c_float, c_void_p],
    "rvc_gate": [c_void_p, c_void_p, c_int64, c_int64, c_int64, c_void_p],
    "rvc_flip_channels": [c_void_p, c_void_p, c_int64, c_int64, c_int64, c_void_p],
    "rvc_transpose": [c_void_p, c_void_p, c_int64, c_int64, c_int64, c_void_p],
    "rvc_randn": [c_void_p, c_int64, c_uint64, c_uint64, c_void_p],
    "rvc_randn_ex": [c_void_p, c_int64, c_uint64, c_uint64, c_void_p, c_void_p],
    "rvc_rand_triang": [c_void_p, c_int64, c_float, c_float, c_uint64, c_uint64, c_void_p, c_void_p],
    "rvc_sine_source": [c_void_p, c_void_p, c_void_p, c_void_p, c_int64, c_int64, c_int, c_float, c_float, c_float,
                        c_void_p],
    "rvc_rand_uniform": [c_void_p, c_int64, c_uint64, c_uint64, c_void_p, c_void_p],
    "rvc_harmonic_source_ws_bytes": [c_int64, c_int64, c_int, c_int],
    "rvc_harmonic_source_chunk": [],
    "rvc_harmonic_source": [c_void_p, c_void_p, c_void_p, c_void_p, c_int64, c_int64, c_int, c_int, c_int, c_float,
                            POINTER(c_float), c_float, c_void_p, c_int64, c_void_p],
    "rvc_upsample_linear": [c_void_p, c_void_p, c_int64, c_int64, c_int64, c_int, c_int64, c_int64, c_int, c_float,
                            c_void_p],
    "rvc_adain": [c_void_p, c_void_p, c_void_p, c_void_p, c_int64, c_int64, c_int64, c_float, c_float, c_int,
                  POINTER(c_uint64), c_uint64, c_void_p, c_void_p],
    "rvc_stft_frames": [c_void_p, c_void_p, c_void_p, c_int64, c_int64, c_int, c_int, c_void_p],
    "rvc_spec_mag": [c_void_p, c_void_p, c_int64, c_int64, c_void_p],
    "rvc_stft_mag": [c_void_p, c_void_p, c_void_p, c_int64, c_int64, c_int64, c_int, c_int, c_int64, c_int64, c_void_p],
    "rvc_mel_image": [c_void_p, c_void_p, c_int64, c_int64, c_int64, c_float, c_float, c_void_p],
    "rvc_avgpool2": [c_void_p, c_void_p, c_int64, c_int64, c_int64, c_void_p],
    "rvc_interleave4": [c_void_p, c_void_p, c_int64, c_int64, c_int64, c_void_p],
    "rvc_img_to_seq": [c_void_p, c_void_p, c_int64, c_int64, c_int64, c_void_p],
    "rvc_bigru": [c_void_p, c_void_p, c_void_p, c_void_p, c_void_p, c_void_p, c_int64, c_void_p],
    "rvc_bigru_set_spin_limit": [ctypes.c_uint],
    "rvc_bigru_batched": [c_void_p, c_int64, c_void_p, c_void_p, c_void_p, c_int64, c_void_p, c_void_p, c_int64, c_int64,
                          c_void_p],
    "rvc_conv64": [POINTER(Conv64Args), c_void_p, c_int64, c_void_p],
    "rvc_conv64_workspace_bytes": [POINTER(Conv64Args)],
    "rvc_conv64_plan": [POINTER(Conv64Args), POINTER(c_int)],
    "rvc_wino64_use": [c_int64, c_int64, c_int64, c_int64],
    "rvc_wino64_weights": [c_void_p, c_void_p, c_int64, c_int64, c_void_p],
    "rvc_wino64_workspace_bytes": [POINTER(Wino64Args)],
# ... 120 lines not shown
```

### rvc-maker_amd/rvc_amd/ops.py

```python
from __future__ import annotations

import ctypes
import math
import os

import torch

from . import _lib
from ._lib import ACT_GELU, ACT_LOGCLAMP, ACT_LRELU, ACT_NONE, ACT_RELU, ACT_SIGMOID, ACT_TANH, check


def _stream():
    return ctypes.c_void_p(torch.cuda.current_stream().cuda_stream)


def _p(t):
    if t is None:
        return None
    if not t.is_cuda or t.dtype not in (torch.float32, torch.int64, torch.int32):
        raise TypeError(f"rvc_amd: expected a CUDA f32/int tensor, got {t.dtype} on {t.device}")
    return ctypes.c_void_p(t.data_ptr())


def pack_km(w: torch.Tensor, groups: int = 1) -> torch.Tensor:
# ... 83 lines not shown
    def for_passes(self, passes):
        return self.hf if passes == F16X3 else self.bf

    def data_ptr(self, passes=None):
        return self.for_passes(PASSES[_PRECISION] if passes is None else passes).data_ptr()


def pack_x6(w_km: torch.Tensor, nphase: int, Ci: int, K: int, Co: int):
    if not X6:
        return None, 0
    lib = _lib.load()
    imgs = []
    for size_fn, pack_fn in ((lib.rvc_conv1d_x6_bytes, lib.rvc_conv1d_pack_x6),
                             (lib.rvc_conv1d_f16_bytes, lib.rvc_conv1d_pack_f16)):
        nbytes = size_fn(nphase, Ci, K, Co)
        if nbytes <= 0:
            raise ValueError("pack_x6: bad shape")
        out = torch.empty(nbytes, dtype=torch.uint8, device=w_km.device)
        nmf = ctypes.c_int(0)
        check(pack_fn(_p(w_km), nphase, Ci, K, Co, ctypes.c_void_p(out.data_ptr()), ctypes.byref(nmf), _stream()),
              "conv1d_pack")
        imgs.append(out)
    return SplitImages(*imgs), nmf.value


class Conv:

    def __init__(self, w, b=None, groups=1, device="cuda"):
        self.Co, self.Cig, self.K = (int(s) for s in w.shape)
        self.groups = groups
        self.Ci = self.Cig * groups
        self.w = pack_km(w.float(), groups).to(device)
        self.b = b.float().to(device) if b is not None else None
        if groups == 1 and self.K <= 64:
            self.wx, self.wx_nmf = pack_x6(self.w, 1, self.Ci, self.K, self.Co)
        elif groups > 1 and self.K <= 128:
            self.wx, self.wx_nmf = pack_x6(self.w, groups, self.Cig, self.K, self.Co // groups)
        else:
            self.wx, self.wx_nmf = None, 0

    def __call__(self, x, Lout=None, stride=1, pad=0, dil=1, **kw):
        return conv1d(x, self.w, self.Ci, self.Co, self.K, bias=self.b, stride=stride, pad=pad, dil=dil,
                      groups=self.groups, Lout=Lout, wx=self.wx, wx_nmf=self.wx_nmf, **kw)


class ConvT:

    def __init__(self, w, b, u, pad, device="cuda"):
        self.Ci, self.Co, self.K = (int(s) for s in w.shape)
        self.u, self.pad = u, pad
        wp, self.T = pack_convT(w.float(), u)
        self.w = wp.to(device)
        self.b = b.float().to(device)
        self.wx, self.wx_nmf = pack_x6(self.w, u, self.Ci, self.T, self.Co)

    def out_len(self, Lin):
        return (Lin - 1) * self.u - 2 * self.pad + self.K

    def __call__(self, x, out=None, **kw):
        B, Ci, Lin = _shape3(x)
        Lout = self.out_len(Lin)
        ncols = (Lout - 1 + self.pad) // self.u + 1
        return conv1d(x, self.w, Ci, self.Co, self.T, bias=self.b, stride=1, pad=self.T - 1, dil=1, Lout=Lout,
                      ncols=ncols, nphase=self.u, ostride=self.u, ooffset=-self.pad, out=out,
                      flops=2.0 * B * Ci * self.Co * self.K * Lin, wx=self.wx, wx_nmf=self.wx_nmf, **kw)


class AmaxSlots:

    def __init__(self, n, device, B=1):
        self.B = B
        self.words = torch.zeros(n * B * AMAX_SHARDS, dtype=torch.int32, device=device)

    def __getitem__(self, k):
        w = self.B * AMAX_SHARDS
        return self.words[k * w:(k + 1) * w]
# ... 31 lines not shown
        return self.store

    def __exit__(self, *a):
        global _WS_PRIVATE
        _WS_PRIVATE = self.prev


def _workspace(device, nbytes, kind="conv"):
    key = f"{device}/{kind}/{torch.cuda.current_stream(device).stream_id}"
    pool = _WS if _WS_PRIVATE is None else _WS_PRIVATE
    buf = pool.get(key)
    if buf is None or buf.numel() * 4 < nbytes:
        if buf is not None and _WS_PRIVATE is not None:
            pool.setdefault("_retired", []).append(buf)
        buf = torch.empty((nbytes + 3) // 4 + (1 << 20), dtype=torch.float32, device=device)
        pool[key] = buf
    return buf


def _room(t):
    return t.untyped_storage().nbytes() // t.element_size() - t.storage_offset()


def _shape3(x):
    if x.dim() == 2:
        return 1, x.shape[0], x.shape[1]
    return x.shape[0], x.shape[1], x.shape[2]


def conv1d(x, w, Ci, Co, K, *, bias=None, bias2=None, stride=1, pad=0, dil=1, groups=1, Lout=None, ncols=0,
           nphase=1, ostride=1, ooffset=0, out=None, res=None, in_act=ACT_NONE, in_slope=0.0, in_scale=1.0,
           out_act=ACT_NONE, out_slope=0.0, out_scale=1.0, accumulate=False, B=None, Lin=None, x_bstride=0,
           w_bstride=0, y_bstride=0, res_bstride=0, toff=None, wrap=0, flops=None, wx=None, wx_nmf=0,
           amax_in=None, amax_out=None, src=None):
    global LAST_CONV_FLOPS, LAST_CONV_ENGINE, LAST_CONV_PASSES, LAST_CONV_WS, _LAST_CONV_ARGS
    if B is None:
        B, Cx, Lx = _shape3(x)
        if Lin is None:
            Lin = Lx
        if Cx != Ci:
            raise ValueError(f"conv1d: x has {Cx} channels, weight expects {Ci}")
        if not x.is_contiguous():
            raise ValueError("conv1d: x must be contiguous")
    if Lout is None:
        Lout = (Lin + 2 * pad - dil * (K - 1) - 1) // stride + 1
    if Lout <= 0:
        raise ValueError("conv1d: empty output")
    Cig = Ci // groups
    need_w = nphase * Cig * K * Co
    if w.numel() < need_w or (w_bstride and w.numel() < need_w + (B - 1) * w_bstride):
        raise ValueError("conv1d: packed weight too small")
    if out is None:
        out = torch.empty(B, Co, Lout, device=x.device, dtype=torch.float32) if B > 1 else \
            torch.empty(Co, Lout, device=x.device, dtype=torch.float32)
    elif _room(out) < (B - 1) * (y_bstride or Co * Lout) + Co * Lout:
        raise ValueError("conv1d: output buffer too small")
    if res is not None and _room(res) < (B - 1) * (res_bstride or Co * Lout) + Co * Lout:
        raise ValueError("conv1d: residual too small")
    if _room(x) < (B - 1) * (x_bstride or Ci * Lin) + Ci * Lin:
        raise ValueError("conv1d: input buffer too small")
    if bias is not None and bias.numel() < Co:
        raise ValueError("conv1d: bias too small")
    a = _lib.Conv1dArgs()
    a.x, a.w, a.bias, a.bias2, a.res, a.y = _p(x), _p(w), _p(bias), _p(bias2), _p(res), _p(out)
    a.B, a.Ci, a.Co, a.Lin, a.Lout, a.ncols = B, Ci, Co, Lin, Lout, ncols
    a.x_bstride, a.y_bstride, a.res_bstride, a.w_bstride = x_bstride, y_bstride, res_bstride, w_bstride
    a.K, a.stride, a.dil, a.pad, a.groups = K, stride, dil, pad, groups
    a.nphase, a.ostride, a.ooffset = nphase, ostride, ooffset
    a.in_act, a.out_act, a.accumulate = in_act, out_act, int(bool(accumulate))
    a.in_scale, a.in_slope, a.out_slope, a.out_scale = in_scale, in_slope, out_slope, out_scale
    if toff is not None:
        if len(toff) != K or K > 16:
            raise ValueError("conv1d: toff must have K <= 16 entries")
        a.ntoff = K
        for i, v in enumerate(toff):
            a.toff[i] = int(v)
    a.wrap = wrap
    a.amax_in, a.amax_out = _p(amax_in), _p(amax_out)
    for cell in (amax_in, amax_out):
        if cell is not None and cell.numel() < B * AMAX_SHARDS:
            raise ValueError(f"conv1d: a |max| cell needs {AMAX_SHARDS} words per batch element (B={B})")
    if src is not None:
        sconv, sig, s_stride, s_pad = src
        if sconv.Ci != 1 or sconv.groups != 1 or sconv.Co != Co:
            raise ValueError("conv1d: src needs a 1-input-channel conv with the output's channels")
        s_len = sig.shape[-1]
        if sig.dim() not in (1, 2) or (sig.dim() == 2 and sig.shape[0] != B) or not sig.is_contiguous() or \
                (sig.dim() == 1 and B != 1):
            raise ValueError("conv1d: src signal must be contiguous [B][N]")
        a.src_x, a.src_w, a.src_b = _p(sig), _p(sconv.w), _p(sconv.b)
        a.src_K, a.src_stride, a.src_pad, a.src_len, a.src_bstride = sconv.K, s_stride, s_pad, s_len, s_len
    if wx is not None:
        passes = conv_passes(K, Ci // groups, stride, toff is not None, amax_in is not None)
        a.wx, a.wx_nmf, a.wx_passes = ctypes.c_void_p(wx.data_ptr(passes)), wx_nmf, passes
    if flops is None:
        valid = (Lout // wrap - 2) * (wrap - 2) if wrap else (ncols or Lout) * nphase
        flops = 2.0 * B * Co * Cig * K * min(valid, Lout)
    LAST_CONV_FLOPS = flops
    lib = _lib.load()
    need = lib.rvc_conv1d_workspace_bytes(ctypes.byref(a))
    if need < 0:
        raise RuntimeError(f"rvc_amd: conv1d plan failed: {lib.rvc_last_error().decode()}")
    ws = _workspace(out.device, need) if need else None
    LAST_CONV_WS = need
    LAST_CONV_ENGINE = lib.rvc_conv1d_engine(ctypes.byref(a))
    LAST_CONV_PASSES = a.wx_passes if LAST_CONV_ENGINE == 1 else 0
    _LAST_CONV_ARGS = a
    check(lib.rvc_conv1d(ctypes.byref(a), _p(ws), need, _stream()), "conv1d")
    return out


FUSED_RB = os.environ.get("RVC_AMD_FUSED_RB", "1") != "0"
RB_PASSES = (6, 3, 1, F16X3)


RB_F16_KMIN = int(os.environ.get("RVC_AMD_RB_F16_KMIN", "3"))


def rb_passes(K):
    if _PRECISION == "fp32" and F16_MIX and K >= RB_F16_KMIN:
        return F16X3
    return PASSES[_PRECISION]


FUSED_RB128 = os.environ.get("RVC_AMD_FUSED_RB128", "0") != "0"


def resblock_fusable(c1: "Conv", c2: "Conv", dil: int) -> bool:
    passes = rb_passes(c1.K)
    chans = c1.Co in (32, 64) or (c1.Co == 128 and FUSED_RB128 and passes in (3, 1, F16X3))
    return (FUSED_RB and passes in RB_PASSES and c1.wx is not None and c2.wx is not None
            and c1.Ci == c1.Co == c2.Ci == c2.Co
            and chans and c1.K == c2.K and c1.K % 2 == 1 and c1.K <= 15 and (c1.K - 1) * dil <= 64)


def resblock_pair(x, y, c1: "Conv", c2: "Conv", dil: int, slope: float, accumulate: bool = False):
    B, C, L = _shape3(x)
    if y.shape != x.shape or not x.is_contiguous() or not y.is_contiguous() or x.data_ptr() == y.data_ptr():
        raise ValueError("resblock_pair: x, y must be distinct contiguous [(B)][C][L] buffers")
    a = _lib.ResblockArgs()
    a.x, a.y = _p(x), _p(y)
    passes = rb_passes(c1.K)
# ... 45 lines not shown
        check(_lib.load().rvc_layernorm_cf(_p(x), _p(res), _p(gamma), _p(beta), _p(out), B, C, T, eps, _stream()),
              "layernorm_cf")
    return out


def chnorm_gelu(x, gamma, beta, out, B, C, L, eps=1e-5, gelu=True):
    if x.numel() < B * C * L or out.numel() < B * C * L:
        raise ValueError("chnorm_gelu: size mismatch")
    check(_lib.load().rvc_chnorm_gelu(_p(x), _p(gamma), _p(beta), _p(out), B, C, L, eps, int(gelu), _stream()),
          "chnorm_gelu")
    return out


def fe0_gn_gelu(wav, w_km, gamma, beta, B, N, C, K, stride, eps=1e-5, gelu=True, x_bstride=0, amax_out=None):
    lib = _lib.load()
    T = (N - K) // stride + 1
    out = torch.empty(B, C, T, device=wav.device) if B > 1 else torch.empty(C, T, device=wav.device)
    need = lib.rvc_fe0_ws_bytes(B, C, T)
    ws = _workspace(wav.device, need, kind="fe0")
    if amax_out is not None and amax_out.numel() < B * AMAX_SHARDS:
        raise ValueError("fe0_gn_gelu: amax_out needs a cell per batch element")
    check(lib.rvc_fe0_gn_gelu_amax(_p(wav), B, N, x_bstride, _p(w_km), C, K, stride, _p(gamma), _p(beta), _p(out),
                                   eps, int(gelu), _p(amax_out), _p(ws), need, _stream()), "fe0_gn_gelu")
    return out


def prior_sample(stats, noise, zp, B, C, T, nscale=0.66666):
    check(_lib.load().rvc_prior_sample(_p(stats), _p(noise), _p(zp), B, C, T, nscale, _stream()), "prior_sample")
    return zp


def gate(a, out, B, H, T):
    check(_lib.load().rvc_gate(_p(a), _p(out), B, H, T, _stream()), "gate")
    return out


def flip_channels(x, out, B, C, T):
    check(_lib.load().rvc_flip_channels(_p(x), _p(out), B, C, T, _stream()), "flip")
    return out


def transpose(x, out, B, R, C):
    check(_lib.load().rvc_transpose(_p(x), _p(out), B, R, C, _stream()), "transpose")
    return out


_DEV_SEED = None


class device_seed:

    def __init__(self, t):
        self.t = t

    def __enter__(self):
        global _DEV_SEED
        self.prev, _DEV_SEED = _DEV_SEED, self.t
        return self

    def __exit__(self, *a):
        global _DEV_SEED
        _DEV_SEED = self.prev


def graph_mode() -> bool:
    return _DEV_SEED is not None
# ... 547 lines not shown
```

### rvc-maker_amd/rvc_amd/synth.py

```python
from __future__ import annotations

import math

import torch

from . import ops
from .ops import ACT_LRELU, ACT_RELU, ACT_TANH, Conv, ConvT

import os

LRELU_SLOPE = 0.1
REFINEGAN_SLOPE = 0.2
MRF_NAMES = ("MRF-HiFi-GAN", "MRF HiFi-GAN")
AMAX = os.environ.get("RVC_AMD_AMAX", "1") != "0"
AMAX_UPS = os.environ.get("RVC_AMD_AMAX_UPS", "1") != "0"
AMAX_PER_STAGE = 16
FUSED_NOISE = os.environ.get("RVC_AMD_FUSED_NOISE", "0") != "0"
ATTN_F16 = os.environ.get("RVC_AMD_ATTN_F16", "1") != "0"
TE_AMAX = os.environ.get("RVC_AMD_TE_AMAX", "0") != "0"
FLOW_AMAX = os.environ.get("RVC_AMD_FLOW_AMAX", "0") != "0"


def fold_weight_norm(weight: dict) -> dict:
    W = {}
    for k, v in weight.items():
        if k.endswith(".weight_v"):
            base = k[: -len(".weight_v")]
            W[base + ".weight"] = torch._weight_norm(v.float(), weight[base + ".weight_g"].float(), 0)
        elif not k.endswith(".weight_g"):
            W[k] = v.float()
    return W


class SynthesizerAMD:
    def __init__(self, cpt: dict, device: str = "cuda"):
        cfg = list(cpt["config"])
        cfg[-3] = cpt["weight"]["emb_g.weight"].shape[0]
        self.cfg = cfg
        (_, _, self.inter, self.hidden, self.filt, self.n_heads, self.n_layers, self.ksz, _, _, self.rks, self.rds,
         self.ur, self.uic, self.uks, self.spk, self.gin, self.sr) = cfg
        self.version = cpt.get("version", "v1")
        self.vocoder = cpt.get("vocoder", "Default")
        if cpt.get("f0", 1) != 1:
            raise NotImplementedError("rvc_amd: only f0 models are on the hot path (the reference's no-f0 Generator "
                                      "does not run)")
        if self.vocoder == "RefineGAN":
            self.kind = "refinegan"
        elif self.vocoder in MRF_NAMES:
            self.kind = "mrf"
        elif self.vocoder == "Default":
            self.kind = "nsf"
        else:
            raise NotImplementedError(f"rvc_amd: vocoder {self.vocoder!r}: Default, MRF-HiFi-GAN and RefineGAN are "
                                      "on the hot path")
        self.upp = math.prod(self.ur)
        self.device = device
        W = fold_weight_norm(cpt["weight"])
        dev = device
        H = self.hidden
        self.kc = H // self.n_heads
        self.emb_dim = W["enc_p.emb_phone.weight"].shape[1]
        self.emb_phone = Conv(W["enc_p.emb_phone.weight"].unsqueeze(-1), W["enc_p.emb_phone.bias"], device=dev)
        self.emb_pitch = W["enc_p.emb_pitch.weight"].contiguous().to(dev)
        self.layers = []
        for i in range(self.n_layers):
            p = f"enc_p.encoder.attn_layers.{i}."
            wqkv = torch.cat([W[p + "conv_q.weight"], W[p + "conv_k.weight"], W[p + "conv_v.weight"]], 0)
            bqkv = torch.cat([W[p + "conv_q.bias"], W[p + "conv_k.bias"], W[p + "conv_v.bias"]], 0)
            ek = W[p + "emb_rel_k"][0]
            L = dict(
                qkv=Conv(wqkv, bqkv, device=dev),
                relk=Conv(ek.unsqueeze(-1), None, device=dev),
                ev=W[p + "emb_rel_v"][0].contiguous().to(dev),
                o=Conv(W[p + "conv_o.weight"], W[p + "conv_o.bias"], device=dev),
                ln1=(W[f"enc_p.encoder.norm_layers_1.{i}.gamma"].to(dev), W[f"enc_p.encoder.norm_layers_1.{i}.beta"].to(dev)),
                ffn1=Conv(W[f"enc_p.encoder.ffn_layers.{i}.conv_1.weight"], W[f"enc_p.encoder.ffn_layers.{i}.conv_1.bias"], device=dev),
                ffn2=Conv(W[f"enc_p.encoder.ffn_layers.{i}.conv_2.weight"], W[f"enc_p.encoder.ffn_layers.{i}.conv_2.bias"], device=dev),
                ln2=(W[f"enc_p.encoder.norm_layers_2.{i}.gamma"].to(dev), W[f"enc_p.encoder.norm_layers_2.{i}.beta"].to(dev)),
            )
            self.layers.append(L)
        self.proj = Conv(W["enc_p.proj.weight"], W["enc_p.proj.bias"], device=dev)
        conds_w = [W[f"flow.flows.{2 * f}.enc.cond_layer.weight"] for f in range(4)] + [W["dec.cond.weight"]]
        conds_b = [W[f"flow.flows.{2 * f}.enc.cond_layer.bias"] for f in range(4)] + [W["dec.cond.bias"]]
        self.cond = Conv(torch.cat(conds_w, 0), torch.cat(conds_b, 0), device=dev)
        self.emb_g = W["emb_g.weight"].contiguous().to(dev)
        self.flows = []
        for f in range(4):
            p = f"flow.flows.{2 * f}."
            F = dict(pre=Conv(W[p + "pre.weight"], W[p + "pre.bias"], device=dev), ins=[], rs_a=[], rs_b=[],
                     post=Conv(W[p + "post.weight"], W[p + "post.bias"], device=dev))
            for l in range(3):
                F["ins"].append(Conv(W[p + f"enc.in_layers.{l}.weight"], W[p + f"enc.in_layers.{l}.bias"], device=dev))
                rw, rb = W[p + f"enc.res_skip_layers.{l}.weight"], W[p + f"enc.res_skip_layers.{l}.bias"]
                if l < 2:
                    F["rs_a"].append(Conv(rw[:H], rb[:H], device=dev))
                    F["rs_b"].append(Conv(rw[H:], rb[H:], device=dev))
                else:
                    F["rs_b"].append(Conv(rw, rb, device=dev))
            self.flows.append(F)
        if self.kind == "refinegan":
            self._load_refinegan(W, dev)
            return
        mrf = self.kind == "mrf"
        if mrf:
            self.n_harm = int(W["dec.m_source.l_linear.weight"].numel())
            self.src_w = [float(v) for v in W["dec.m_source.l_linear.weight"].reshape(-1)]
            self.src_linear = False
        else:
            self.n_harm = 1
            self.lin_w = float(W["dec.m_source.l_linear.weight"].reshape(-1)[0])
        self.lin_b = float(W["dec.m_source.l_linear.bias"].reshape(-1)[0])
        self.conv_pre = Conv(W["dec.conv_pre.weight"], W["dec.conv_pre.bias"], device=dev)
        nup = len(self.ur)
        self.chans = [self.uic // (2 ** (i + 1)) for i in range(nup)]
        strides = [math.prod(self.ur[i + 1:]) if i + 1 < nup else 1 for i in range(nup)]
        self.ups, self.noise, self.res = [], [], []
        ups_name = "dec.upsamples" if mrf else "dec.ups"
        for i, (u, k) in enumerate(zip(self.ur, self.uks)):
            if u % 2:
                raise NotImplementedError("odd upsample rates (output_padding) are not used by any shipped config")
            self.ups.append(ConvT(W[f"{ups_name}.{i}.weight"], W[f"{ups_name}.{i}.bias"], u, (k - u) // 2, device=dev))
            s = strides[i]
            kn = 1 if s == 1 else s * 2 - s % 2
            self.noise.append((Conv(W[f"dec.noise_convs.{i}.weight"], W[f"dec.noise_convs.{i}.bias"], device=dev), s,
                               0 if s == 1 else (kn - s) // 2))
            blocks = []
            for j, (kk, ds) in enumerate(zip(self.rks, self.rds)):
                if mrf:
                    rb = f"dec.mrfs.{i}.{j}.layers."
# ... 84 lines not shown
                          k_hs=kc * T, v_hs=kc * T, o_hs=kc * T, q_bs=3 * H * T, k_bs=3 * H * T, v_bs=3 * H * T,
                          o_bs=H * T, scale=scale, rk=rk, ev=L["ev"], ml=ml, W=10,
                          amax_in=c_qkv, amax_out=c_o)
            y = L["o"](o, out=tmp, amax_in=c_o)
            ops.layernorm_cf(x, y, L["ln1"][0], L["ln1"][1], x, B, H, T, amax_out=c_l1)
            h = L["ffn1"](x, pad=(self.ksz - 1) // 2, out_act=ACT_RELU, amax_in=c_l1, amax_out=c_f1)
            y = L["ffn2"](h, pad=(self.ksz - 1) // 2, out=tmp, amax_in=c_f1)
            ops.layernorm_cf(x, y, L["ln2"][0], L["ln2"][1], x, B, H, T, amax_out=c_l2)
            x_cell = c_l2
        return self.proj(x, amax_in=x_cell).view(B, 2 * self.inter, T)

    def flow_reverse(self, z_p, gc, T, B=1):
        H, I, half, dev = self.hidden, self.inter, self.inter // 2, z_p.device
        x = z_p
        bufs = (torch.empty(B, I, T, device=dev), torch.empty(B, I, T, device=dev))
        h = torch.empty(B, H, T, device=dev)
        acts = torch.empty(B, H, T, device=dev)
        out_acc = torch.empty(B, H, T, device=dev)
        cells = ops.AmaxSlots(1 + 5 * 4, dev, B) if FLOW_AMAX else None
        cell = (lambda k: cells[k]) if cells is not None else (lambda k: None)
        if cells is not None:
            cells[0].view(B, ops.AMAX_SHARDS)[:, 0].fill_(0x3F800000)
        unit = cell(0)
        post_cell = None
        for n, f in enumerate(reversed(range(4))):
            F = self.flows[f]
            c_h = [cell(1 + 5 * n + k) for k in range(3)]
            c_acc, c_post = cell(1 + 5 * n + 3), cell(1 + 5 * n + 4)
            xf = bufs[0] if x is not bufs[0] else bufs[1]
            ops.flip_channels(x, xf, B, I, T)
            F["pre"](xf, B=B, Lin=T, x_bstride=I * T, out=h, amax_in=post_cell, amax_out=c_h[0])
            for l in range(3):
                g_l = gc[f * 6 * H + l * 2 * H: f * 6 * H + (l + 1) * 2 * H]
                xin = F["ins"][l](h, pad=2, bias2=g_l, amax_in=c_h[l])
                ops.gate(xin, acts, B, H, T)
                if l < 2:
                    F["rs_a"][l](acts, out=h, res=h, amax_in=unit, amax_out=c_h[l + 1])
                    F["rs_b"][l](acts, out=out_acc, accumulate=(l > 0), amax_in=unit)
                else:
                    F["rs_b"][l](acts, out=out_acc, accumulate=True, amax_in=unit, amax_out=c_acc)
            x1 = xf[:, half:]
            F["post"](out_acc, out=x1, res=x1, y_bstride=I * T, res_bstride=I * T, out_scale=-1.0, amax_in=c_acc,
                      amax_out=c_post)
            post_cell = c_post
            x = xf
        return x

    def harmonic_source(self, nsff0, sine_noise, phase0, T, B=1):
        har = torch.empty(B, T * self.upp, device=nsff0.device)
        return ops.harmonic_source(nsff0, phase0, sine_noise, har, B, T, self.upp, self.n_harm, float(self.sr),
                                   self.src_w, self.lin_b, linear=self.src_linear)

    def generator(self, z, nsff0, gdec, T, sine_noise, B=1, phase0=None):
        dev = z.device
        L = T * self.upp
        if self.kind == "mrf":
            har = self.harmonic_source(nsff0, sine_noise, phase0, T, B)
        else:
            har = torch.empty(B, L, device=dev)
            work = torch.empty(B, T, device=dev)
            ops.sine_source(nsff0, sine_noise, har, work, B, T, self.upp, float(self.sr), self.lin_w, self.lin_b)
        nst = len(self.ur)
        cells = ops.AmaxSlots(AMAX_PER_STAGE * nst + nst + 1, dev, B) if AMAX else None
        out_cell = (lambda k: cells[AMAX_PER_STAGE * nst + k]) if AMAX else (lambda k: None)
        x = self.conv_pre(z.reshape(B, self.inter, T), pad=3, bias2=gdec, amax_out=out_cell(nst))
        x_cell = out_cell(nst)
        scale = 1.0
        nk = len(self.rks)
        for i in range(nst):
# ... 220 lines not shown
```

Measured before the change: 1186 audio-s/s.

## Fuse flow WaveNet gate and res-skip split into conv epilogues; fold attention combine

Adds conv output modes that apply the tanh·sigmoid gate directly in the in_layer conv epilogue, using interleaved weight rows, and that write the res_skip conv to two destinations (residual-updated h and the accumulated skip buffer) from a single launch. This replaces a separate gate kernel and two res_skip convs per flow layer. Attention also gets an option to fold the split-KV combine into the relative-position band kernel, which drops a launch and one round trip of the output through memory. The cost is more template variants, including split-K reduce variants, and an extra probe call on every layer. The dual-output path is skipped when flow amax cells are enabled.

Measured after the change: 1189 audio-s/s, median of 6. Within noise of the previous version (+0.3%).

```diff
diff --git a/include/rvc_amd.h b/include/rvc_amd.h
--- a/include/rvc_amd.h
+++ b/include/rvc_amd.h
@@ -59,6 +59,20 @@
 int rvc_conv1d_engine(const rvc_conv1d_args* a);
 int rvc_conv1d_tile(const rvc_conv1d_args* a);
 int rvc_conv1d(const rvc_conv1d_args* a, void* ws, int64_t ws_bytes, rvc_stream_t stream);
+
+#define RVC_CONV_OUT_PLAIN 0
+#define RVC_CONV_OUT_GATE 1
+#define RVC_CONV_OUT_DUAL 2
+typedef struct rvc_conv1d_ext {
+    int mode;
+    int accumulate2;
+    int64_t split_row;
+    float* y2;
+    int64_t y2_bstride;
+} rvc_conv1d_ext;
+int rvc_conv1d_ext_ok(const rvc_conv1d_args* a, const rvc_conv1d_ext* e);
+int rvc_conv1d_ex(const rvc_conv1d_args* a, const rvc_conv1d_ext* e, void* ws, int64_t ws_bytes, rvc_stream_t stream);
+int rvc_gate_rows(int64_t H, int64_t* perm);
 void rvc_conv1d_set_probe_event(void* hip_event);
 int rvc_conv1d_set_stamps(void* buf, int64_t bytes);
 int rvc_resblock_set_stamps(void* buf, int64_t bytes);
@@ -115,6 +129,8 @@
 int rvc_attention_ex(const rvc_attn_args* a, const unsigned* amax_in, unsigned* amax_out, void* ws, int64_t ws_bytes,
                      rvc_stream_t stream);
 int rvc_attention_set_f16(int on);
+int rvc_attention_set_band_combine(int on);
+int rvc_attention_set_splits(int splits);
 
 int rvc_textenc_embed(const float* lin, const float* emb, const int64_t* pitch, float* out, int64_t B, int64_t C,
                       int64_t T, float scale, float slope, rvc_stream_t stream);
@@ -136,6 +152,7 @@
 int rvc_prior_sample(const float* stats, const float* noise, float* zp, int64_t B, int64_t C, int64_t T, float nscale,
                      rvc_stream_t stream);
 int rvc_gate(const float* a, float* out, int64_t B, int64_t H, int64_t T, rvc_stream_t stream);
+int rvc_gate_il(const float* a, float* out, int64_t B, int64_t H, int64_t T, rvc_stream_t stream);
 int rvc_flip_channels(const float* x, float* out, int64_t B, int64_t C, int64_t T, rvc_stream_t stream);
 int rvc_transpose(const float* in, float* out, int64_t B, int64_t R, int64_t C, rvc_stream_t stream);
 int rvc_randn(float* out, int64_t n, uint64_t seed, uint64_t offset, rvc_stream_t stream);
diff --git a/rvc-maker_amd/csrc/attention.hip b/rvc-maker_amd/csrc/attention.hip
--- a/rvc-maker_amd/csrc/attention.hip
+++ b/rvc-maker_amd/csrc/attention.hip
@@ -480,13 +480,22 @@
     }
 }
 
+__device__ __forceinline__ float mul_rounded(float a, float b) {
+#pragma clang fp contract(off)
+    return a * b;
+}
+
 constexpr int RELV_QB = 32, RELV_KW = RELV_QB + 2 * 15;
+constexpr int RELV_SMAX = 32;
+template <bool COMBINE>
 __global__ __launch_bounds__(256) void attn_relv_band_kernel(AttnParams p, const float* ev, int D) {
     constexpr int QB = RELV_QB;
     __shared__ float pb[QB][32];
     __shared__ float evs[31 * 96];
     __shared__ float qs[96][QB + 1];
     __shared__ float ks[96][RELV_KW + 1];
+    __shared__ float cw[COMBINE ? RELV_SMAX : 1][QB];
+    __shared__ float cm[2][QB];
     const int h = blockIdx.y, b = blockIdx.z;
     const int64_t T = p.T;
     const int64_t q0 = (int64_t)blockIdx.x * QB;
@@ -495,8 +504,30 @@
     const float* Q = p.q + b * p.q_bs + h * p.q_hs;
     const float* K = p.k + b * p.k_bs + h * p.k_hs;
     const float* RK = p.rk + ((int64_t)b * p.H + h) * nb * T;
-    const float* ML = p.ml + ((int64_t)b * p.H + h) * 2 * T;
+    float* ML = p.ml + ((int64_t)b * p.H + h) * 2 * T;
     float* O = p.o + b * p.o_bs + h * p.o_hs;
+    const int S = p.S;
+    if constexpr (COMBINE) {
+        if (tid < QB) {
+            const int64_t qa = q0 + tid < T ? q0 + tid : T - 1;
+            const float* wml = p.ws + (int64_t)gridDim.z * S * p.H * D * T;
+            float m = -INFINITY;
+            for (int s = 0; s < S; ++s) m = fmaxf(m, wml[(((int64_t)b * S + s) * p.H + h) * 2 * T + qa]);
+            float wsum = 0.f;
+            for (int s = 0; s < S; ++s) {
+                const int64_t bsh = ((int64_t)b * S + s) * p.H + h;
+                const float l = wml[bsh * 2 * T + T + qa], e = expf(wml[bsh * 2 * T + qa] - m);
+                wsum = fmaf(l, e, wsum);
+                cw[s][tid] = mul_rounded(l, e);
+            }
+            cm[0][tid] = m;
+            cm[1][tid] = wsum;
+            if (q0 + tid < T) {
+                ML[qa] = m;
+                ML[T + qa] = wsum;
+            }
+        }
+    }
     for (int i = tid; i < nb * D; i += 256) evs[i] = ev[i];
     for (int i = tid; i < D * QB; i += 256) {
         const int c = i / QB, qi = i - c * QB;
@@ -509,6 +540,26 @@
         ks[c][ji] = (j >= 0 && j < T) ? K[(int64_t)c * p.ldc + j] : 0.f;
     }
     __syncthreads();
+    constexpr int NK = 96 * QB / 256;
+    float oc[COMBINE ? NK : 1];
+    if constexpr (COMBINE) {
+        const int qi = tid & (QB - 1), c0 = tid >> 5;
+        const int64_t qa = q0 + qi < T ? q0 + qi : T - 1;
+#pragma unroll
+        for (int k = 0; k < NK; ++k) oc[k] = 0.f;
+        for (int s = 0; s < S; ++s) {
+            const float w = cw[s][qi];
+            const float* wo = p.ws + (((int64_t)b * S + s) * p.H + h) * D * T + qa;
+#pragma unroll
+            for (int k = 0; k < NK; ++k) {
+                const int c = c0 + 8 * k;
+                oc[k] = fmaf(w, wo[(int64_t)(c < D ? c : D - 1) * T], oc[k]);
+            }
+        }
+        const float inv = 1.f / cm[1][qi];
+#pragma unroll
+        for (int k = 0; k < NK; ++k) oc[k] = mul_rounded(oc[k], inv);
+    }
     for (int i = tid; i < QB * nb; i += 256) {
         const int qi = i % QB, r = i / QB;
         const int64_t qa = q0 + qi, j = qa + r - p.W;
@@ -517,30 +568,50 @@
             float sc = 0.f;
             for (int c = 0; c < D; ++c) sc += (qs[c][qi] * p.scale) * ks[c][qi + r];
             sc += RK[(int64_t)r * T + qa];
-            pv = expf(sc - ML[qa]) / ML[T + qa];
+            if constexpr (COMBINE) pv = expf(sc - cm[0][qi]) / cm[1][qi];
+            else pv = expf(sc - ML[qa]) / ML[T + qa];
         }
         pb[qi][r] = pv;
     }
     __syncthreads();
     float amx = 0.f;
-    for (int i = tid; i < QB * D; i += 256) {
-        const int qi = i % QB, c = i / QB;
+    if constexpr (COMBINE) {
+        const int qi = tid & (QB - 1), c0 = tid >> 5;
         const int64_t qa = q0 + qi;
-        if (qa >= T) continue;
-        float acc = 0.f;
-        for (int r = 0; r < nb; ++r) acc += pb[qi][r] * evs[r * D + c];
-        const float v = O[(int64_t)c * p.ldc + qa] + acc;
-        O[(int64_t)c * p.ldc + qa] = v;
-        amx = fmaxf(amx, fabsf(v));
+#pragma unroll
+        for (int k = 0; k < NK; ++k) {
+            const int c = c0 + 8 * k;
+            if (qa < T && c < D) {
+                float acc = 0.f;
+                for (int r = 0; r < nb; ++r) acc += pb[qi][r] * evs[r * D + c];
+                const float v = oc[k] + acc;
+                O[(int64_t)c * p.ldc + qa] = v;
+                amx = fmaxf(amx, fabsf(v));
+            }
+        }
+    } else {
+        for (int i = tid; i < QB * D; i += 256) {
+            const int qi = i % QB, c = i / QB;
+            const int64_t qa = q0 + qi;
+            if (qa >= T) continue;
+            float acc = 0.f;
+            for (int r = 0; r < nb; ++r) acc += pb[qi][r] * evs[r * D + c];
+            const float v = O[(int64_t)c * p.ldc + qa] + acc;
+            O[(int64_t)c * p.ldc + qa] = v;
+            amx = fmaxf(amx, fabsf(v));
+        }
     }
     if (p.amax_out) amax_publish_block(p.amax_out + (int64_t)b * RVC_AMAX_SHARDS, amx);
 }
+
+thread_local int g_attn_splits = 0;
 
 void attn_plan(const rvc_attn_args* a, int& S, int& kps, int qpb = 64) {
     const int64_t blocks = (int64_t)cdiv(a->T, qpb) * a->H * a->B;
     int64_t s = (512 + blocks - 1) / blocks;
     const int64_t smax = a->T / 256;
     if (s > smax) s = smax;
+    if (g_attn_splits > 0) s = g_attn_splits;
     if (s > 32) s = 32;
     if (s < 1) s = 1;
     kps = (int)((a->T + s - 1) / s + 63) / 64 * 64;
@@ -571,6 +642,18 @@
 
 extern "C" int rvc_attention_set_f16(int on) {
     g_attn_f16 = on < 0 ? -1 : (on ? 1 : 0);
+    return RVC_OK;
+}
+
+static thread_local int g_band_combine = -1;
+
+extern "C" int rvc_attention_set_band_combine(int on) {
+    g_band_combine = on < 0 ? -1 : (on ? 1 : 0);
+    return RVC_OK;
+}
+
+extern "C" int rvc_attention_set_splits(int splits) {
+    g_attn_splits = splits > 0 ? splits : 0;
     return RVC_OK;
 }
 
@@ -610,16 +693,20 @@
     } else if (a->D == 64) hipLaunchKernelGGL(attn_fwd_kernel<64>, grid, dim3(256), 0, s, p);
     else hipLaunchKernelGGL(attn_fwd_kernel<96>, grid, dim3(256), 0, s, p);
     RVC_HIP(hipGetLastError());
-    if (p.S > 1) {
+    static const int bc_env = getenv("RVC_ATTN_BAND_COMBINE") ? atoi(getenv("RVC_ATTN_BAND_COMBINE")) : 1;
+    const bool band = a->rk && a->ev;
+    const bool fold = band && p.S > 1 && (g_band_combine >= 0 ? g_band_combine : bc_env);
+    if (p.S > 1 && !fold) {
         const dim3 cg(cdiv(a->T, 64), (unsigned)a->H, (unsigned)a->B);
         if (a->D == 64) hipLaunchKernelGGL(attn_combine_kernel<64>, cg, dim3(256), 0, s, p);
         else hipLaunchKernelGGL(attn_combine_kernel<96>, cg, dim3(256), 0, s, p);
         RVC_HIP(hipGetLastError());
     }
-    if (a->rk && a->ev) {
+    if (band) {
         p.amax_out = amax_out;
-        hipLaunchKernelGGL(attn_relv_band_kernel, dim3(cdiv(a->T, 32), (unsigned)a->H, (unsigned)a->B), dim3(256), 0,
-                           s, p, a->ev, a->D);
+        const dim3 bg(cdiv(a->T, RELV_QB), (unsigned)a->H, (unsigned)a->B);
+        if (fold) hipLaunchKernelGGL(attn_relv_band_kernel<true>, bg, dim3(256), 0, s, p, a->ev, (int)a->D);
+        else hipLaunchKernelGGL(attn_relv_band_kernel<false>, bg, dim3(256), 0, s, p, a->ev, (int)a->D);
         RVC_HIP(hipGetLastError());
     }
     return RVC_OK;
diff --git a/rvc-maker_amd/csrc/conv1d.hip b/rvc-maker_amd/csrc/conv1d.hip
--- a/rvc-maker_amd/csrc/conv1d.hip
+++ b/rvc-maker_amd/csrc/conv1d.hip
@@ -41,6 +41,10 @@
     int stagger_blocks;
     int swz;
     int gx6;
+    int omode;
+    int split_row, accumulate2;
+    float* y2;
+    int64_t y2_bstride;
 #if RVC_CONV_STAMPS
     unsigned long long* stamps;
     int64_t stamp_blocks;
@@ -186,6 +190,87 @@
             }
     }
     if (p.amax_out) amax_publish(p.amax_out + (int64_t)b * RVC_AMAX_SHARDS, amx);
+}
+
+template <int FM, int FN, int WM, int WN, bool TB, int MODE>
+__device__ __forceinline__ void conv_epilogue_ext(const ConvParams& p, floatx4 (&acc)[FM][FN], int lane, int wm, int wn,
+                                                  int b, int Cog, int m0g, int64_t n0, const float* tb) {
+    static_assert(MODE == RVC_CONV_OUT_GATE || MODE == RVC_CONV_OUT_DUAL, "an output mode");
+    static_assert(MODE != RVC_CONV_OUT_GATE || FM % 2 == 0, "gate: row fragments in pairs");
+    constexpr int BM = 16 * FM * WM;
+    const int ln = lane & 15;
+    const int lr = (lane >> 4) * 4;
+    int tcol[FN];
+#pragma unroll
+    for (int j = 0; j < FN; ++j) tcol[j] = out_pos(p, n0 + wn * 16 * FN + j * 16 + ln, 0);
+    const int Lo = (int)p.Lout;
+    if constexpr (MODE == RVC_CONV_OUT_GATE) {
+        float* yb = p.y + b * p.y_bstride;
+#pragma unroll
+        for (int i = 0; i < FM; i += 2) {
+#pragma unroll
+            for (int r = 0; r < 4; ++r) {
+                const int rl = wm * 16 * FM + i * 16 + lr + r;
+                const int mg = m0g + rl;
+                const bool mok = mg < Cog;
+                const float bsa = epi_bias<TB, BM>(p, tb, rl, mok ? mg : 0);
+                const float bsb = epi_bias<TB, BM>(p, tb, rl + 16, mok ? mg + 16 : 0);
+                const int orow = (mg >> 5) * 16 + (mg & 15);
+#pragma unroll
+                for (int j = 0; j < FN; ++j) {
+                    float xa = acc[i][j][r], xb = acc[i + 1][j][r];
+                    xa += bsa;
+                    xb += bsb;
+                    const float v = gate_apply(xa, xb);
+                    if (mok && tcol[j] >= 0) yb[orow * Lo + tcol[j]] = v;
+                }
+            }
+        }
+    } else {
+#pragma unroll
+        for (int i = 0; i < FM; ++i) {
+            floatx4 (&av)[1][FN] = *reinterpret_cast<floatx4 (*)[1][FN]>(&acc[i][0]);
+            const bool second = m0g + wm * 16 * FM + i * 16 >= p.split_row;
+            const int roff = second ? p.split_row : 0;
+            float* yb = second ? p.y2 + b * p.y2_bstride : p.y + b * p.y_bstride;
+            const float* rb2 = !second && p.res ? p.res + b * p.res_bstride : nullptr;
+            const bool accum = second ? p.accumulate2 != 0 : p.accumulate != 0;
+            int mrow[4], orow[4];
+            bool mok[4];
+#pragma unroll
+            for (int r = 0; r < 4; ++r) {
+                const int mg = m0g + wm * 16 * FM + i * 16 + lr + r;
+                mok[r] = mg < Cog;
+                mrow[r] = mg < Cog ? mg : roff;
+                orow[r] = mrow[r] - roff;
+                const float bs = epi_bias<TB, BM>(p, tb, wm * 16 * FM + i * 16 + lr + r, mrow[r]);
+#pragma unroll
+                for (int j = 0; j < FN; ++j) av[0][j][r] += bs;
+            }
+            switch (p.out_act) {
+                case RVC_ACT_LRELU: apply_act<RVC_ACT_LRELU, 1, FN>(av, p.out_slope, p.out_scale); break;
+                case RVC_ACT_RELU: apply_act<RVC_ACT_RELU, 1, FN>(av, p.out_slope, p.out_scale); break;
+                default: apply_act<RVC_ACT_NONE, 1, FN>(av, p.out_slope, p.out_scale); break;
+            }
+            if (rb2) {
+#pragma unroll
+                for (int r = 0; r < 4; ++r)
+#pragma unroll
+                    for (int j = 0; j < FN; ++j) av[0][j][r] += rb2[orow[r] * Lo + (tcol[j] >= 0 ? tcol[j] : 0)];
+            }
+            if (accum) {
+#pragma unroll
+                for (int r = 0; r < 4; ++r)
+#pragma unroll
+                    for (int j = 0; j < FN; ++j) av[0][j][r] += yb[orow[r] * Lo + (tcol[j] >= 0 ? tcol[j] : 0)];
+            }
+#pragma unroll
+            for (int r = 0; r < 4; ++r)
+#pragma unroll
+                for (int j = 0; j < FN; ++j)
+                    if (mok[r] && tcol[j] >= 0) yb[orow[r] * Lo + tcol[j]] = av[0][j][r];
+        }
+    }
 }
 
 template <int FM, int FN, int WM, int WN>
@@ -424,7 +509,7 @@
     if (p.amax_out) amax_publish(p.amax_out + (int64_t)b * RVC_AMAX_SHARDS, amx);
 }
 
-template <int FM, int FN, int WM, int WN>
+template <int FM, int FN, int WM, int WN, int MODE = 0>
 __global__ __launch_bounds__(256) void conv1d_mfma_kernel(ConvParams p) {
     constexpr int BM = 16 * FM * WM;
     constexpr int BN = 16 * FN * WN;
@@ -601,7 +686,12 @@
         __syncthreads();
     }
 
-    conv_epilogue<FM, FN, WM, WN>(p, acc, lane, wm, wn, split, phase, b, g, Cog, m0g, n0);
+    if constexpr (MODE != 0) {
+        if (p.ksplit > 1) conv_store_partial<FM, FN, WM, WN>(p, acc, lane, wm, wn, split, phase, b, g, Cog, m0g, n0);
+        else conv_epilogue_ext<FM, FN, WM, WN, false, MODE>(p, acc, lane, wm, wn, b, Cog, m0g, n0, nullptr);
+    } else {
+        conv_epilogue<FM, FN, WM, WN>(p, acc, lane, wm, wn, split, phase, b, g, Cog, m0g, n0);
+    }
 }
 
 constexpr int X6_NI_MAX = 6;
@@ -724,8 +814,11 @@
     if (p.amax_out && !part) amax_publish(p.amax_out + (int64_t)b * RVC_AMAX_SHARDS, amx);
 }
 
-template <int FM, int FN, int WM, int WN, int X6_NI, int NP, bool F16, bool SA = false, int LF = 0>
+template <int FM, int FN, int WM, int WN, int X6_NI, int NP, bool F16, bool SA = false, int LFM = 0>
 __global__ __launch_bounds__(64 * (WM * WN + 4), (x6_min_blocks<FM, FN, WM * WN, NP>())) void conv_x6_kernel(ConvParams p) {
+    constexpr int LF = LFM > 0 ? LFM : 0;
+    constexpr int MODE = LFM < 0 ? -LFM : 0;
+    static_assert(MODE == 0 || (NP == 6 && !F16 && !SA && FN != 8), "output modes: the 6-pass split-bf16 128-wide tiles");
     static_assert(WM * WN == 4 || WM * WN == 8, "4 or 8 compute waves");
     constexpr int NCW = WM * WN;
     static_assert(NP == 6 || NP == 3 || NP == 1, "6, 3 or 1 passes");
@@ -1157,7 +1250,10 @@
                 for (int j = 0; j < FN; ++j) acc[i][j][r] *= f;
             }
     }
-    if (BN <= 128 && p.tile_epi) {
+    if constexpr (MODE != 0) {
+        if (p.ksplit > 1) conv_store_partial<FM, FN, WM, WN>(p, acc, lane, wm, wn, split, ophase, b, grp, Cog, m0g, n0);
+        else conv_epilogue_ext<FM, FN, WM, WN, true, MODE>(p, acc, lane, wm, wn, b, Cog, m0g, n0, etab);
+    } else if (BN <= 128 && p.tile_epi) {
         float* ot = reinterpret_cast<float*>(xs);
         constexpr int TS = BN + 4;
 #pragma unroll
@@ -1289,6 +1385,97 @@
         }
     }
     if (p.amax_out) amax_publish_block(p.amax_out + (int64_t)b * RVC_AMAX_SHARDS, amx);
+}
+
+template <int MODE>
+__global__ __launch_bounds__(256) void conv_splitk_reduce_ext(ConvParams p) {
+    const int64_t n = (int64_t)blockIdx.x * blockDim.x + threadIdx.x;
+    const int b = blockIdx.z;
+    const int64_t m0 = (int64_t)blockIdx.y * RED_ROWS;
+    const bool okn = n < p.ncols;
+    const int t = okn ? out_pos(p, n, 0) : -1;
+    const bool ok = t >= 0;
+    const int64_t Lo = p.Lout;
+    const int64_t sstride = p.B * p.Co * p.ncols;
+    if constexpr (MODE == RVC_CONV_OUT_GATE) {
+        const int64_t ma = (m0 >> 4) * 32 + (m0 & 15);
+        const float* src = p.ws + ((int64_t)b * p.Co + ma) * p.ncols + (okn ? n : 0);
+        float sa[RED_ROWS], sb[RED_ROWS];
+#pragma unroll
+        for (int r = 0; r < RED_ROWS; ++r) sa[r] = sb[r] = 0.f;
+        for (int k = 0; k < p.ksplit; ++k) {
+            float va[RED_ROWS], vb[RED_ROWS];
+#pragma unroll
+            for (int r = 0; r < RED_ROWS; ++r) {
+                va[r] = src[k * sstride + (int64_t)r * p.ncols];
+                vb[r] = src[k * sstride + (int64_t)(r + 16) * p.ncols];
+            }
+#pragma unroll
+            for (int r = 0; r < RED_ROWS; ++r) {
+                sa[r] += va[r];
+                sb[r] += vb[r];
+            }
+        }
+        float* yb = p.y + b * p.y_bstride;
+#pragma unroll
+        for (int r = 0; r < RED_ROWS; ++r) {
+            float xa = sa[r], xb = sb[r];
+            if (p.bias) {
+                xa += p.bias[ma + r];
+                xb += p.bias[ma + 16 + r];
+            }
+            if (p.bias2) {
+                xa += p.bias2[ma + r];
+                xb += p.bias2[ma + 16 + r];
+            }
+            const float v = gate_apply(xa, xb);
+            if (ok) yb[(m0 + r) * Lo + t] = v;
+        }
+    } else {
+        const bool second = m0 >= p.split_row;
+        const int64_t ro = m0 - (second ? p.split_row : 0);
+        const int nr = p.Co - m0 < RED_ROWS ? (int)(p.Co - m0) : RED_ROWS;
+        const float* src = p.ws + ((int64_t)b * p.Co + m0) * p.ncols + (okn ? n : 0);
+        float s[RED_ROWS];
+#pragma unroll
+        for (int r = 0; r < RED_ROWS; ++r) s[r] = 0.f;
+        for (int k = 0; k < p.ksplit; ++k) {
+            float v[RED_ROWS];
+#pragma unroll
+            for (int r = 0; r < RED_ROWS; ++r) v[r] = src[k * sstride + (int64_t)(r < nr ? r : nr - 1) * p.ncols];
+#pragma unroll
+            for (int r = 0; r < RED_ROWS; ++r) s[r] += v[r];
+        }
+        float v[RED_ROWS];
+        int64_t o[RED_ROWS];
+#pragma unroll
+        for (int r = 0; r < RED_ROWS; ++r) {
+            const int rc = r < nr ? r : nr - 1;
+            o[r] = (ro + rc) * Lo + (ok ? t : 0);
+            float x = s[r];
+            if (p.bias) x += p.bias[m0 + rc];
+            if (p.bias2) x += p.bias2[m0 + rc];
+            v[r] = act_apply(x, p.out_act, p.out_slope) * p.out_scale;
+        }
+        if (!second && p.res) {
+            float rr[RED_ROWS];
+#pragma unroll
+            for (int r = 0; r < RED_ROWS; ++r) rr[r] = p.res[b * p.res_bstride + o[r]];
+#pragma unroll
+            for (int r = 0; r < RED_ROWS; ++r) v[r] += rr[r];
+        }
+        float* yb = second ? p.y2 + b * p.y2_bstride : p.y + b * p.y_bstride;
+        if (second ? p.accumulate2 : p.accumulate) {
+            float aa[RED_ROWS];
+#pragma unroll
+            for (int r = 0; r < RED_ROWS; ++r) aa[r] = yb[o[r]];
+#pragma unroll
+            for (int r = 0; r < RED_ROWS; ++r) v[r] += aa[r];
+        }
+#pragma unroll
+        for (int r = 0; r < RED_ROWS; ++r)
+            if (r < nr && ok) yb[o[r]] = v[r];
+    }
 }
 
 struct SrcParams {
@@ -1439,6 +1626,10 @@
     static const int swz_env = getenv("RVC_X6_SWZ") ? atoi(getenv("RVC_X6_SWZ")) : 1;
     p.swz = g_swz >= 0 ? g_swz : swz_env;
     p.gx6 = 0;
+    p.omode = 0;
+    p.split_row = p.accumulate2 = 0;
+    p.y2 = nullptr;
+    p.y2_bstride = 0;
 #if RVC_CONV_STAMPS
     p.stamps = g_stamps;
     p.stamp_blocks = g_stamp_blocks;
@@ -1509,7 +1700,7 @@
                                                 a->wx_passes == 1 || a->wx_passes == RVC_ARITH_F16X3);
 }
 
-int plan(const rvc_conv1d_args* a, ConvParams& p, Cfg& cfg, dim3& grid, size_t& lds) {
+int plan(const rvc_conv1d_args* a, ConvParams& p, Cfg& cfg, dim3& grid, size_t& lds, const rvc_conv1d_ext* e = nullptr) {
     RVC_CHECK_ARG(a && a->x && a->w && a->y, "conv1d: null pointer");
     RVC_CHECK_ARG(a->B > 0 && a->Ci > 0 && a->Co > 0 && a->K > 0 && a->Lin > 0 && a->Lout > 0,
                   "conv1d: bad sizes B=%lld Ci=%lld Co=%lld K=%d Lin=%lld Lout=%lld", (long long)a->B,
@@ -1522,6 +1713,32 @@
     const int64_t Cig = a->Ci / a->groups;
     const int64_t ncols = a->ncols > 0 ? a->ncols : a->Lout;
     fill_common(a, p);
+    if (e && e->mode != RVC_CONV_OUT_PLAIN) {
+        RVC_CHECK_ARG(e->mode == RVC_CONV_OUT_GATE || e->mode == RVC_CONV_OUT_DUAL, "conv1d: unknown output mode %d", e->mode);
+        RVC_CHECK_ARG(a->groups == 1 && a->nphase == 1 && a->ostride == 1 && a->ooffset == 0 && !a->wrap && !a->ntoff &&
+                          !a->src_x && !a->amax_out && a->w_bstride == 0,
+                      "conv1d: an output mode takes a plain 1-D conv (one group, one phase, no |max| cell, no source)");
+        p.omode = e->mode;
+        if (e->mode == RVC_CONV_OUT_GATE) {
+            RVC_CHECK_ARG(a->Co % 32 == 0 && !a->res && !a->accumulate && a->out_act == RVC_ACT_NONE &&
+                              a->out_scale == 1.f,
+                          "conv1d: gate mode needs Co %% 32 == 0 (Co=%lld) and no residual / accumulate / activation / scale",
+                          (long long)a->Co);
+            p.y_bstride = a->y_bstride ? a->y_bstride : a->Co / 2 * a->Lout;
+        } else {
+            RVC_CHECK_ARG(e->y2 && e->split_row > 0 && e->split_row < a->Co && e->split_row % 16 == 0,
+                          "conv1d: dual mode needs y2 and 0 < split_row < Co, a multiple of 16 (split_row=%lld)",
+                          (long long)e->split_row);
+            RVC_CHECK_ARG(a->out_act == RVC_ACT_NONE || a->out_act == RVC_ACT_LRELU || a->out_act == RVC_ACT_RELU,
+                          "conv1d: dual mode takes no transcendental activation");
+            p.split_row = (int)e->split_row;
+            p.accumulate2 = e->accumulate2;
+            p.y2 = e->y2;
+            p.y_bstride = a->y_bstride ? a->y_bstride : e->split_row * a->Lout;
+            p.res_bstride = a->res_bstride ? a->res_bstride : e->split_row * a->Lout;
+            p.y2_bstride = e->y2_bstride ? e->y2_bstride : (a->Co - e->split_row) * a->Lout;
+        }
+    }
     RVC_CHECK_ARG(!a->src_x || (a->src_w && a->src_K > 0 && a->src_K <= 4096 && a->src_stride > 0 && a->src_pad >= 0 &&
                                 a->src_len > 0 && a->src_bstride >= 0 && !a->wrap),
                   "conv1d: bad fused source conv (src_K=%d src_stride=%d src_pad=%d src_len=%lld)", a->src_K,
@@ -1585,7 +1802,7 @@
         const size_t tile_bytes = (size_t)BM * (BN + 4) * 4;
         const bool plain = a->nphase == 1 && a->ostride == 1 && a->ooffset == 0 && !a->wrap && !(p.dbg & 1) &&
                            BN <= 128;
-        p.tile_epi = !(tepi && plain && a->groups == 1) ? 0
+        p.tile_epi = !(tepi && plain && a->groups == 1 && !p.omode) ? 0
                      : tile_bytes <= lds ? 1 : (cfg.WM % 2 == 0 && tile_bytes / 2 <= lds) ? 2 : 0;
         lds += (size_t)3 * BM * 4;
         grid = dim3(cdiv(ncols, BN), (unsigned)p.mtiles_per_group, (unsigned)(a->B * p.nphase * p.ksplit));
@@ -1822,13 +2039,91 @@
 #endif
 }
 
-extern "C" int rvc_conv1d(const rvc_conv1d_args* a, void* ws, int64_t ws_bytes, rvc_stream_t stream) {
+namespace {
+
+bool ext_cfg_ok(const ConvParams& p, const Cfg& cfg) {
+    if (!cfg.x6) return cfg.FM == 2 || cfg.FM == 4;
+    const bool tile = (cfg.FM == 2 && cfg.FN == 4 && cfg.WM == 4 && cfg.WN == 2) ||
+                      (cfg.FM == 2 && cfg.FN == 2 && cfg.WM == 2 && cfg.WN == 4) ||
+                      (cfg.FM == 2 && cfg.FN == 2 && cfg.WM == 1 && cfg.WN == 4);
+    return tile && p.wx_passes == 6 && 4 * p.span <= 256 * 3 && !p.gx6;
+}
+
+template <int FM, int FN, int WM, int WN>
+hipError_t launch_x6_ext(const ConvParams& p, dim3 grid, size_t lds, hipStream_t s) {
+    const dim3 blk(64 * (WM * WN + 4));
+    if (p.omode == RVC_CONV_OUT_GATE)
+        hipLaunchKernelGGL((conv_x6_kernel<FM, FN, WM, WN, 3, 6, false, false, -RVC_CONV_OUT_GATE>), grid, blk, lds, s, p);
+    else hipLaunchKernelGGL((conv_x6_kernel<FM, FN, WM, WN, 3, 6, false, false, -RVC_CONV_OUT_DUAL>), grid, blk, lds, s, p);
+    return hipGetLastError();
+}
+
+template <int FM, int FN, int WM, int WN>
+hipError_t launch_ext(const ConvParams& p, dim3 grid, size_t lds, hipStream_t s) {
+    if (p.omode == RVC_CONV_OUT_GATE)
+        hipLaunchKernelGGL((conv1d_mfma_kernel<FM, FN, WM, WN, RVC_CONV_OUT_GATE>), grid, dim3(256), lds, s, p);
+    else hipLaunchKernelGGL((conv1d_mfma_kernel<FM, FN, WM, WN, RVC_CONV_OUT_DUAL>), grid, dim3(256), lds, s, p);
+    return hipGetLastError();
+}
+
+int conv1d_run_ext(const ConvParams& p, const Cfg& cfg, dim3 grid, size_t lds, hipStream_t s, hipEvent_t probe) {
+    hipError_t e;
+    if (cfg.x6) {
+        if (cfg.WM == 4) e = launch_x6_ext<2, 4, 4, 2>(p, grid, lds, s);
+        else if (cfg.WM == 2) e = launch_x6_ext<2, 2, 2, 4>(p, grid, lds, s);
+        else e = launch_x6_ext<2, 2, 1, 4>(p, grid, lds, s);
+    } else if (cfg.WM == 1 && cfg.FN == 4) e = launch_ext<2, 4, 1, 4>(p, grid, lds, s);
+    else if (cfg.WM == 1) e = launch_ext<2, 2, 1, 4>(p, grid, lds, s);
+    else if (cfg.FM == 4 && cfg.FN == 4) e = launch_ext<4, 4, 2, 2>(p, grid, lds, s);
+    else if (cfg.FM == 4) e = launch_ext<4, 2, 2, 2>(p, grid, lds, s);
+    else if (cfg.FN == 4) e = launch_ext<2, 4, 2, 2>(p, grid, lds, s);
+    else e = launch_ext<2, 2, 2, 2>(p, grid, lds, s);
+    RVC_HIP(e);
+    if (probe) RVC_HIP(hipEventRecord(probe, s));
+    if (p.ksplit > 1) {
+        if (p.omode == RVC_CONV_OUT_GATE)
+            hipLaunchKernelGGL(conv_splitk_reduce_ext<RVC_CONV_OUT_GATE>,
+                               dim3(cdiv(p.ncols, 256), (unsigned)(p.Co / 2 / RED_ROWS), (unsigned)p.B), dim3(256), 0, s, p);
+        else
+            hipLaunchKernelGGL(conv_splitk_reduce_ext<RVC_CONV_OUT_DUAL>,
+                               dim3(cdiv(p.ncols, 256), (unsigned)cdiv(p.Co, RED_ROWS), (unsigned)p.B), dim3(256), 0, s, p);
+        RVC_HIP(hipGetLastError());
+    }
+    return RVC_OK;
+}
+
+}
+
+extern "C" int rvc_gate_rows(int64_t H, int64_t* perm) {
+    RVC_CHECK_ARG(perm && H > 0 && H % 16 == 0, "gate_rows: H %% 16 == 0 (H=%lld)", (long long)H);
+    for (int64_t p = 0; p < 2 * H; ++p) perm[p] = ((p >> 4) & 1) * H + (p >> 5) * 16 + (p & 15);
+    return RVC_OK;
+}
+
+extern "C" int rvc_conv1d_ext_ok(const rvc_conv1d_args* a, const rvc_conv1d_ext* e) {
     ConvParams p;
     Cfg cfg;
     dim3 grid;
     size_t lds;
-    int rc = plan(a, p, cfg, grid, lds);
+    if (!e || e->mode == RVC_CONV_OUT_PLAIN) return 0;
+    if (plan(a, p, cfg, grid, lds, e) != RVC_OK) return -1;
+    return ext_cfg_ok(p, cfg) ? 1 : 0;
+}
+
+extern "C" int rvc_conv1d(const rvc_conv1d_args* a, void* ws, int64_t ws_bytes, rvc_stream_t stream) {
+    return rvc_conv1d_ex(a, nullptr, ws, ws_bytes, stream);
+}
+
+extern "C" int rvc_conv1d_ex(const rvc_conv1d_args* a, const rvc_conv1d_ext* ext, void* ws, int64_t ws_bytes,
+                             rvc_stream_t stream) {
+    ConvParams p;
+    Cfg cfg;
+    dim3 grid;
+    size_t lds;
+    int rc = plan(a, p, cfg, grid, lds, ext);
     if (rc != RVC_OK) return rc;
+    RVC_CHECK_ARG(!p.omode || ext_cfg_ok(p, cfg), "conv1d: output mode %d is not compiled for this call's plan (ask "
+                                                  "rvc_conv1d_ext_ok first)", p.omode);
     if (p.ksplit > 1) {
         const int64_t need = (int64_t)p.ksplit * p.B * p.nphase * p.Co * p.ncols * 4;
         RVC_CHECK_ARG(ws && ws_bytes >= need, "conv1d: split-K needs %lld B of workspace (got %lld)",
@@ -1836,6 +2131,7 @@
         p.ws = (float*)ws;
     }
     hipStream_t s = (hipStream_t)stream;
+    if (p.omode) return conv1d_run_ext(p, cfg, grid, lds, s, g_probe_event);
     if (a->src_x) p.amax_out = nullptr;
     hipError_t e;
     if (cfg.x6) {
diff --git a/rvc-maker_amd/csrc/elementwise.hip b/rvc-maker_amd/csrc/elementwise.hip
--- a/rvc-maker_amd/csrc/elementwise.hip
+++ b/rvc-maker_amd/csrc/elementwise.hip
@@ -142,6 +142,24 @@
     return RVC_OK;
 }
 
+__global__ void gate_il_kernel(const float* a, float* out, int H, int64_t T) {
+    int64_t t = (int64_t)blockIdx.x * blockDim.x + threadIdx.x;
+    int c = blockIdx.y, b = blockIdx.z;
+    if (t >= T) return;
+    const float* ab = a + (int64_t)b * 2 * H * T;
+    const int ra = (c >> 4) * 32 + (c & 15);
+    float x0 = ab[(int64_t)ra * T + t], x1 = ab[(int64_t)(ra + 16) * T + t];
+    out[((int64_t)b * H + c) * T + t] = tanhf(x0) * (1.f / (1.f + expf(-x1)));
+}
+
+extern "C" int rvc_gate_il(const float* a, float* out, int64_t B, int64_t H, int64_t T, rvc_stream_t stream) {
+    RVC_CHECK_ARG(a && out && B > 0 && H > 0 && H % 16 == 0 && T > 0, "gate_il: bad args (H %% 16 == 0)");
+    hipLaunchKernelGGL(gate_il_kernel, dim3(cdiv(T, 256), (unsigned)H, (unsigned)B), dim3(256), 0, (hipStream_t)stream,
+                       a, out, (int)H, T);
+    RVC_HIP(hipGetLastError());
+    return RVC_OK;
+}
+
 __global__ void flip_kernel(const float* x, float* out, int C, int64_t T) {
     int64_t t = (int64_t)blockIdx.x * blockDim.x + threadIdx.x;
     int c = blockIdx.y, b = blockIdx.z;
diff --git a/rvc-maker_amd/csrc/model_common.h b/rvc-maker_amd/csrc/model_common.h
--- a/rvc-maker_amd/csrc/model_common.h
+++ b/rvc-maker_amd/csrc/model_common.h
@@ -55,6 +55,8 @@
     bool attn_f16 = true;
     bool te_amax = false;
     bool flow_amax = false;
+    bool flow_gate = true;
+    bool flow_rs = true;
     Synth* syn = nullptr;
     ContentVec* cv = nullptr;
     Rmvpe* rm = nullptr;
@@ -337,11 +339,18 @@
     const float* src_x = nullptr;
     int src_stride = 1, src_pad = 0;
     int64_t src_len = 0;
-};
-
-inline int conv(rvc_ctx* c, ModelBase& m, const ConvW& cw, const float* x, int64_t Lin, float* y, const CallOpts& o,
-                hipStream_t s) {
-    rvc_conv1d_args a;
+    int omode = RVC_CONV_OUT_PLAIN, accumulate2 = 0;
+    int64_t split_row = 0;
+    float* y2 = nullptr;
+};
+
+inline void conv_args(rvc_ctx* c, const ConvW& cw, const float* x, int64_t Lin, float* y, const CallOpts& o,
+                      rvc_conv1d_args& a, rvc_conv1d_ext& e) {
+    memset(&e, 0, sizeof(e));
+    e.mode = o.omode;
+    e.accumulate2 = o.accumulate2;
+    e.split_row = o.split_row;
+    e.y2 = o.y2;
     memset(&a, 0, sizeof(a));
     a.x = x;
     a.w = cw.w;
@@ -406,9 +415,24 @@
         a.wx_nmf = cw.nmf;
         a.wx_passes = passes;
     }
+}
+
+inline bool conv_ext_ok(rvc_ctx* c, const ConvW& cw, const float* x, int64_t Lin, float* y, const CallOpts& o) {
+    rvc_conv1d_args a;
+    rvc_conv1d_ext e;
+    conv_args(c, cw, x, Lin, y, o, a, e);
+    return rvc_conv1d_ext_ok(&a, &e) == 1;
+}
+
+inline int conv(rvc_ctx* c, ModelBase& m, const ConvW& cw, const float* x, int64_t Lin, float* y, const CallOpts& o,
+                hipStream_t s) {
+    rvc_conv1d_args a;
+    rvc_conv1d_ext e;
+    conv_args(c, cw, x, Lin, y, o, a, e);
     const int64_t need = rvc_conv1d_workspace_bytes(&a);
     if (need < 0) return RVC_EINVAL;
     MTRY(ensure_ws(m, need, s));
+    if (e.mode != RVC_CONV_OUT_PLAIN) return rvc_conv1d_ex(&a, &e, need ? m.ws : nullptr, need, s);
     return rvc_conv1d(&a, need ? m.ws : nullptr, need, s);
 }
 
diff --git a/rvc-maker_amd/csrc/rvc_common.h b/rvc-maker_amd/csrc/rvc_common.h
--- a/rvc-maker_amd/csrc/rvc_common.h
+++ b/rvc-maker_amd/csrc/rvc_common.h
@@ -24,6 +24,8 @@
         default: return v;
     }
 }
+
+RVC_DEV float gate_apply(float a, float b) { return tanhf(a) * (1.f / (1.f + expf(-b))); }
 
 RVC_DEV float wave_sum(float v) {
 #pragma unroll
diff --git a/rvc-maker_amd/csrc/rvc_model.cpp b/rvc-maker_amd/csrc/rvc_model.cpp
--- a/rvc-maker_amd/csrc/rvc_model.cpp
+++ b/rvc-maker_amd/csrc/rvc_model.cpp
@@ -1,3 +1,5 @@
+#include <algorithm>
+
 #include "model_common.h"
 
 using namespace rvcm;
@@ -19,6 +21,7 @@
 struct Flow {
     ConvW pre, post;
     ConvW ins[3], rs_a[2], rs_b[3];
+    ConvW rs[2];
 };
 
 }
@@ -31,6 +34,7 @@
     int64_t n_spk = 0;
     std::vector<synthm::Layer> layers;
     synthm::Flow flows[4];
+    bool flow_gate = false, flow_rs = false;
     float lin_w = 0, lin_b = 0;
     std::vector<ConvW> ups;
     std::vector<ConvW> noise;
@@ -247,9 +251,23 @@
             oi.pad = (F.ins[l].K - 1) / 2;
             oi.bias2 = gc + (int64_t)f * 6 * H + (int64_t)l * 2 * H;
             oi.amax_in = c_h[l];
-            MTRY(conv(c, S, F.ins[l], h, T, xin, oi, s));
-            MTRY(rvc_gate(xin, acts, 1, H, T, s));
-            if (l < 2) {
+            CallOpts og = oi;
+            og.omode = RVC_CONV_OUT_GATE;
+            if (S.flow_gate && conv_ext_ok(c, F.ins[l], h, T, acts, og)) {
+                MTRY(conv(c, S, F.ins[l], h, T, acts, og, s));
+            } else {
+                MTRY(conv(c, S, F.ins[l], h, T, xin, oi, s));
+                MTRY((S.flow_gate ? rvc_gate_il : rvc_gate)(xin, acts, 1, H, T, s));
+            }
+            CallOpts rd;
+            rd.res = h;
+            rd.omode = RVC_CONV_OUT_DUAL;
+            rd.split_row = H;
+            rd.y2 = outacc;
+            rd.accumulate2 = l > 0;
+            if (l < 2 && S.flow_rs && !c->flow_amax && conv_ext_ok(c, F.rs[l], acts, T, h, rd)) {
+                MTRY(conv(c, S, F.rs[l], acts, T, h, rd, s));
+            } else if (l < 2) {
                 CallOpts ra;
                 ra.res = h;
                 ra.amax_in = unit;
@@ -437,6 +455,8 @@
     c->attn_f16 = env_on("RVC_AMD_ATTN_F16");
     c->te_amax = env_set("RVC_AMD_TE_AMAX");
     c->flow_amax = env_set("RVC_AMD_FLOW_AMAX");
+    c->flow_gate = env_on("RVC_AMD_FLOW_GATE");
+    c->flow_rs = env_on("RVC_AMD_FLOW_RS");
     *out = c;
     return RVC_OK;
 }
@@ -579,6 +599,17 @@
     GET("enc_p.proj.bias", b);
     MTRY(expect(w, "enc_p.proj.weight", 2 * g.inter_channels, H, 1));
     MTRY(make_conv(c, S, w, &b, S.proj));
+    S.flow_gate = c->flow_gate && H % 16 == 0;
+    S.flow_rs = c->flow_rs;
+    std::vector<int64_t> grow(2 * H);
+    for (int64_t i = 0; i < 2 * H; ++i) grow[i] = i;
+    if (S.flow_gate) MTRY(rvc_gate_rows(H, grow.data()));
+    auto gate_order = [&](HostT& t, int64_t row0) {
+        const int64_t inner = (int64_t)t.v.size() / t.dim(0);
+        const std::vector<float> old(t.v.begin() + row0 * inner, t.v.begin() + (row0 + 2 * H) * inner);
+        for (int64_t p = 0; p < 2 * H; ++p)
+            std::copy(old.begin() + grow[p] * inner, old.begin() + (grow[p] + 1) * inner, t.v.begin() + (row0 + p) * inner);
+    };
     {
         HostT cw, cb;
         for (int f = 0; f <= 4; ++f) {
@@ -586,6 +617,13 @@
             GET(p + "weight", w);
             GET(p + "bias", b);
             MTRY(expect(w, p + "weight", f < 4 ? 2 * H * 3 : g.upsample_initial_channel, g.gin_channels, 1));
+            if (f < 4) {
+                MCHECK((int64_t)b.v.size() == 6 * H, "rvc_load_synth: %sbias has %zu values", p.c_str(), b.v.size());
+                for (int l = 0; l < 3; ++l) {
+                    gate_order(w, (int64_t)l * 2 * H);
+                    gate_order(b, (int64_t)l * 2 * H);
+                }
+            }
             if (f == 0) {
                 cw = w;
                 cb = b;
@@ -618,6 +656,10 @@
             GET(p + "enc.in_layers." + sl + ".weight", w);
             GET(p + "enc.in_layers." + sl + ".bias", b);
             MTRY(expect(w, p + "enc.in_layers." + sl + ".weight", 2 * H, H, 5));
+            MCHECK((int64_t)b.v.size() == 2 * H, "rvc_load_synth: %senc.in_layers.%d.bias has %zu values", p.c_str(), l,
+                   b.v.size());
+            gate_order(w, 0);
+            gate_order(b, 0);
             MTRY(make_conv(c, S, w, &b, F.ins[l]));
             GET(p + "enc.res_skip_layers." + sl + ".weight", w);
             GET(p + "enc.res_skip_layers." + sl + ".bias", b);
@@ -633,6 +675,7 @@
                 bb.v.assign(b.v.begin() + H, b.v.end());
                 MTRY(make_conv(c, S, wa, &ba, F.rs_a[l]));
                 MTRY(make_conv(c, S, wb, &bb, F.rs_b[l]));
+                if (S.flow_rs) MTRY(make_conv(c, S, w, &b, F.rs[l]));
             } else {
                 MTRY(make_conv(c, S, w, &b, F.rs_b[l]));
             }
diff --git a/rvc-maker_amd/rvc_amd/_lib.py b/rvc-maker_amd/rvc_amd/_lib.py
--- a/rvc-maker_amd/rvc_amd/_lib.py
+++ b/rvc-maker_amd/rvc_amd/_lib.py
@@ -28,6 +28,14 @@
                 ("src_len", c_int64), ("src_bstride", c_int64)]
 
 
+CONV_OUT_PLAIN, CONV_OUT_GATE, CONV_OUT_DUAL = 0, 1, 2
+
+
+class Conv1dExt(ctypes.Structure):
+    _fields_ = [("mode", c_int), ("accumulate2", c_int), ("split_row", c_int64), ("y2", c_void_p),
+                ("y2_bstride", c_int64)]
+
+
 class Conv64Args(ctypes.Structure):
     _fields_ = [("x", c_void_p), ("w", c_void_p), ("bias", c_void_p), ("res", c_void_p), ("y", c_void_p),
                 ("B", c_int64), ("Ci", c_int64), ("Co", c_int64), ("Lin", c_int64), ("Lout", c_int64),
@@ -119,6 +127,9 @@
     "rvc_last_error": [],
     "rvc_version": [],
     "rvc_conv1d": [POINTER(Conv1dArgs), c_void_p, c_int64, c_void_p],
+    "rvc_conv1d_ex": [POINTER(Conv1dArgs), POINTER(Conv1dExt), c_void_p, c_int64, c_void_p],
+    "rvc_conv1d_ext_ok": [POINTER(Conv1dArgs), POINTER(Conv1dExt)],
+    "rvc_gate_rows": [c_int64, c_void_p],
     "rvc_conv1d_workspace_bytes": [POINTER(Conv1dArgs)],
     "rvc_conv1d_set_probe_event": [c_void_p],
     "rvc_conv1d_set_stamps": [c_void_p, c_int64],
@@ -167,6 +178,8 @@
     "rvc_attention_amax": [POINTER(AttnArgs), c_void_p, c_void_p, c_int64, c_void_p],
     "rvc_attention_ex": [POINTER(AttnArgs), c_void_p, c_void_p, c_void_p, c_int64, c_void_p],
     "rvc_attention_set_f16": [c_int],
+    "rvc_attention_set_band_combine": [c_int],
+    "rvc_attention_set_splits": [c_int],
     "rvc_layernorm_cf_amax": [c_void_p, c_void_p, c_void_p, c_void_p, c_void_p, c_int64, c_int64, c_int64, c_float,
                               c_void_p, c_void_p],
     "rvc_textenc_embed": [c_void_p, c_void_p, c_void_p, c_void_p, c_int64, c_int64, c_int64, c_float, c_float,
@@ -183,6 +196,7 @@
                              c_void_p, c_float, c_int, c_void_p, c_void_p, c_int64, c_void_p],
     "rvc_prior_sample": [c_void_p, c_void_p, c_void_p, c_int64, c_int64, c_int64, c_float, c_void_p],
     "rvc_gate": [c_void_p, c_void_p, c_int64, c_int64, c_int64, c_void_p],
+    "rvc_gate_il": [c_void_p, c_void_p, c_int64, c_int64, c_int64, c_void_p],
     "rvc_flip_channels": [c_void_p, c_void_p, c_int64, c_int64, c_int64, c_void_p],
     "rvc_transpose": [c_void_p, c_void_p, c_int64, c_int64, c_int64, c_void_p],
     "rvc_randn": [c_void_p, c_int64, c_uint64, c_uint64, c_void_p],
diff --git a/rvc-maker_amd/rvc_amd/ops.py b/rvc-maker_amd/rvc_amd/ops.py
--- a/rvc-maker_amd/rvc_amd/ops.py
+++ b/rvc-maker_amd/rvc_amd/ops.py
@@ -139,6 +139,7 @@
         self.Ci = self.Cig * groups
         self.w = pack_km(w.float(), groups).to(device)
         self.b = b.float().to(device) if b is not None else None
+        self._ext_ok = {}
         if groups == 1 and self.K <= 64:
             self.wx, self.wx_nmf = pack_x6(self.w, 1, self.Ci, self.K, self.Co)
         elif groups > 1 and self.K <= 128:
@@ -149,6 +150,17 @@
     def __call__(self, x, Lout=None, stride=1, pad=0, dil=1, **kw):
         return conv1d(x, self.w, self.Ci, self.Co, self.K, bias=self.b, stride=stride, pad=pad, dil=dil,
                       groups=self.groups, Lout=Lout, wx=self.wx, wx_nmf=self.wx_nmf, **kw)
+
+    def ext_ok(self, x, Lout=None, stride=1, pad=0, dil=1, **kw):
+        key = (bool(kw.get("gate")), kw.get("out2") is not None, kw.get("split_row", 0), tuple(x.shape), kw.get("B"),
+               kw.get("Lin"), Lout, stride, pad, dil, kw.get("amax_in") is not None, kw.get("amax_out") is not None,
+               kw.get("res") is not None, bool(kw.get("accumulate")), _PRECISION)
+        ok = self._ext_ok.get(key)
+        if ok is None:
+            ok = self._ext_ok[key] = _conv1d(x, self.w, self.Ci, self.Co, self.K, bias=self.b, stride=stride, pad=pad,
+                                             dil=dil, groups=self.groups, Lout=Lout, wx=self.wx, wx_nmf=self.wx_nmf,
+                                             probe=True, **kw)
+        return ok
 
 
 class ConvT:
@@ -246,7 +258,8 @@
            nphase=1, ostride=1, ooffset=0, out=None, res=None, in_act=ACT_NONE, in_slope=0.0, in_scale=1.0,
            out_act=ACT_NONE, out_slope=0.0, out_scale=1.0, accumulate=False, B=None, Lin=None, x_bstride=0,
            w_bstride=0, y_bstride=0, res_bstride=0, toff=None, wrap=0, flops=None, wx=None, wx_nmf=0,
-           amax_in=None, amax_out=None, src=None):
+           amax_in=None, amax_out=None, src=None, gate=False, out2=None, split_row=0, accumulate2=False, y2_bstride=0,
+           probe=False):
     global LAST_CONV_FLOPS, LAST_CONV_ENGINE, LAST_CONV_PASSES, LAST_CONV_WS, _LAST_CONV_ARGS
     if B is None:
         B, Cx, Lx = _shape3(x)
@@ -264,12 +277,27 @@
     need_w = nphase * Cig * K * Co
     if w.numel() < need_w or (w_bstride and w.numel() < need_w + (B - 1) * w_bstride):
         raise ValueError("conv1d: packed weight too small")
+    ext = None
+    Cy = Co
+    if gate or out2 is not None:
+        if gate and out2 is not None:
+            raise ValueError("conv1d: gate and out2 are different output modes")
+        ext = _lib.Conv1dExt()
+        if gate:
+            ext.mode, Cy = _lib.CONV_OUT_GATE, Co // 2
+        else:
+            if not 0 < split_row < Co:
+                raise ValueError("conv1d: out2 needs 0 < split_row < Co")
+            if _room(out2) < (B - 1) * (y2_bstride or (Co - split_row) * Lout) + (Co - split_row) * Lout:
+                raise ValueError("conv1d: second output buffer too small")
+            ext.mode, Cy = _lib.CONV_OUT_DUAL, split_row
+            ext.split_row, ext.accumulate2, ext.y2, ext.y2_bstride = split_row, int(bool(accumulate2)), _p(out2), y2_bstride
     if out is None:
-        out = torch.empty(B, Co, Lout, device=x.device, dtype=torch.float32) if B > 1 else \
-            torch.empty(Co, Lout, device=x.device, dtype=torch.float32)
-    elif _room(out) < (B - 1) * (y_bstride or Co * Lout) + Co * Lout:
+        out = torch.empty(B, Cy, Lout, device=x.device, dtype=torch.float32) if B > 1 else \
+            torch.empty(Cy, Lout, device=x.device, dtype=torch.float32)
+    elif _room(out) < (B - 1) * (y_bstride or Cy * Lout) + Cy * Lout:
         raise ValueError("conv1d: output buffer too small")
-    if res is not None and _room(res) < (B - 1) * (res_bstride or Co * Lout) + Co * Lout:
+    if res is not None and _room(res) < (B - 1) * (res_bstride or Cy * Lout) + Cy * Lout:
         raise ValueError("conv1d: residual too small")
     if _room(x) < (B - 1) * (x_bstride or Ci * Lin) + Ci * Lin:
         raise ValueError("conv1d: input buffer too small")
@@ -310,8 +338,10 @@
     if flops is None:
         valid = (Lout // wrap - 2) * (wrap - 2) if wrap else (ncols or Lout) * nphase
         flops = 2.0 * B * Co * Cig * K * min(valid, Lout)
+    lib = _lib.load()
+    if probe:
+        return ext is not None and lib.rvc_conv1d_ext_ok(ctypes.byref(a), ctypes.byref(ext)) == 1
     LAST_CONV_FLOPS = flops
-    lib = _lib.load()
     need = lib.rvc_conv1d_workspace_bytes(ctypes.byref(a))
     if need < 0:
         raise RuntimeError(f"rvc_amd: conv1d plan failed: {lib.rvc_last_error().decode()}")
@@ -320,8 +350,21 @@
     LAST_CONV_ENGINE = lib.rvc_conv1d_engine(ctypes.byref(a))
     LAST_CONV_PASSES = a.wx_passes if LAST_CONV_ENGINE == 1 else 0
     _LAST_CONV_ARGS = a
-    check(lib.rvc_conv1d(ctypes.byref(a), _p(ws), need, _stream()), "conv1d")
-    return out
+    if ext is not None:
+        check(lib.rvc_conv1d_ex(ctypes.byref(a), ctypes.byref(ext), _p(ws), need, _stream()), "conv1d")
+    else:
+        check(lib.rvc_conv1d(ctypes.byref(a), _p(ws), need, _stream()), "conv1d")
+    return out
+
+
+_conv1d = conv1d
+
+
+def gate_rows(H: int) -> torch.Tensor:
+    import numpy as np
+    perm = np.zeros(2 * H, np.int64)
+    check(_lib.load().rvc_gate_rows(H, ctypes.c_void_p(perm.ctypes.data)), "gate_rows")
+    return torch.from_numpy(perm)
 
 
 FUSED_RB = os.environ.get("RVC_AMD_FUSED_RB", "1") != "0"
@@ -433,6 +476,11 @@
 
 def gate(a, out, B, H, T):
     check(_lib.load().rvc_gate(_p(a), _p(out), B, H, T, _stream()), "gate")
+    return out
+
+
+def gate_il(a, out, B, H, T):
+    check(_lib.load().rvc_gate_il(_p(a), _p(out), B, H, T, _stream()), "gate_il")
     return out
 
 
diff --git a/rvc-maker_amd/rvc_amd/synth.py b/rvc-maker_amd/rvc_amd/synth.py
--- a/rvc-maker_amd/rvc_amd/synth.py
+++ b/rvc-maker_amd/rvc_amd/synth.py
@@ -19,6 +19,8 @@
 ATTN_F16 = os.environ.get("RVC_AMD_ATTN_F16", "1") != "0"
 TE_AMAX = os.environ.get("RVC_AMD_TE_AMAX", "0") != "0"
 FLOW_AMAX = os.environ.get("RVC_AMD_FLOW_AMAX", "0") != "0"
+FLOW_GATE = os.environ.get("RVC_AMD_FLOW_GATE", "1") != "0"
+FLOW_RS = os.environ.get("RVC_AMD_FLOW_RS", "1") != "0"
 
 
 def fold_weight_norm(weight: dict) -> dict:
@@ -80,21 +82,28 @@
             )
             self.layers.append(L)
         self.proj = Conv(W["enc_p.proj.weight"], W["enc_p.proj.bias"], device=dev)
-        conds_w = [W[f"flow.flows.{2 * f}.enc.cond_layer.weight"] for f in range(4)] + [W["dec.cond.weight"]]
-        conds_b = [W[f"flow.flows.{2 * f}.enc.cond_layer.bias"] for f in range(4)] + [W["dec.cond.bias"]]
+        self.flow_gate = FLOW_GATE and H % 16 == 0
+        self.flow_rs = FLOW_RS
+        grow = ops.gate_rows(H) if self.flow_gate else torch.arange(2 * H)
+        crow = torch.cat([l * 2 * H + grow for l in range(3)])
+        conds_w = [W[f"flow.flows.{2 * f}.enc.cond_layer.weight"][crow] for f in range(4)] + [W["dec.cond.weight"]]
+        conds_b = [W[f"flow.flows.{2 * f}.enc.cond_layer.bias"][crow] for f in range(4)] + [W["dec.cond.bias"]]
         self.cond = Conv(torch.cat(conds_w, 0), torch.cat(conds_b, 0), device=dev)
         self.emb_g = W["emb_g.weight"].contiguous().to(dev)
         self.flows = []
         for f in range(4):
             p = f"flow.flows.{2 * f}."
-            F = dict(pre=Conv(W[p + "pre.weight"], W[p + "pre.bias"], device=dev), ins=[], rs_a=[], rs_b=[],
+            F = dict(pre=Conv(W[p + "pre.weight"], W[p + "pre.bias"], device=dev), ins=[], rs_a=[], rs_b=[], rs=[],
                      post=Conv(W[p + "post.weight"], W[p + "post.bias"], device=dev))
             for l in range(3):
-                F["ins"].append(Conv(W[p + f"enc.in_layers.{l}.weight"], W[p + f"enc.in_layers.{l}.bias"], device=dev))
+                F["ins"].append(Conv(W[p + f"enc.in_layers.{l}.weight"][grow], W[p + f"enc.in_layers.{l}.bias"][grow],
+                                     device=dev))
                 rw, rb = W[p + f"enc.res_skip_layers.{l}.weight"], W[p + f"enc.res_skip_layers.{l}.bias"]
                 if l < 2:
                     F["rs_a"].append(Conv(rw[:H], rb[:H], device=dev))
                     F["rs_b"].append(Conv(rw[H:], rb[H:], device=dev))
+                    if self.flow_rs:
+                        F["rs"].append(Conv(rw, rb, device=dev))
                 else:
                     F["rs_b"].append(Conv(rw, rb, device=dev))
             self.flows.append(F)
@@ -245,9 +254,16 @@
             F["pre"](xf, B=B, Lin=T, x_bstride=I * T, out=h, amax_in=post_cell, amax_out=c_h[0])
             for l in range(3):
                 g_l = gc[f * 6 * H + l * 2 * H: f * 6 * H + (l + 1) * 2 * H]
-                xin = F["ins"][l](h, pad=2, bias2=g_l, amax_in=c_h[l])
-                ops.gate(xin, acts, B, H, T)
-                if l < 2:
+                ins = F["ins"][l]
+                if self.flow_gate and ins.ext_ok(h, pad=2, bias2=g_l, amax_in=c_h[l], gate=True, out=acts):
+                    ins(h, pad=2, bias2=g_l, amax_in=c_h[l], gate=True, out=acts)
+                else:
+                    xin = ins(h, pad=2, bias2=g_l, amax_in=c_h[l])
+                    (ops.gate_il if self.flow_gate else ops.gate)(xin, acts, B, H, T)
+                if l < 2 and self.flow_rs and cells is None and F["rs"][l].ext_ok(
+                        acts, out=h, res=h, out2=out_acc, split_row=H, accumulate2=(l > 0)):
+                    F["rs"][l](acts, out=h, res=h, out2=out_acc, split_row=H, accumulate2=(l > 0))
+                elif l < 2:
                     F["rs_a"][l](acts, out=h, res=h, amax_in=unit, amax_out=c_h[l + 1])
                     F["rs_b"][l](acts, out=out_acc, accumulate=(l > 0), amax_in=unit)
                 else:
```
